# chenruduan/OAReactDiff

Hardware: AMD Instinct MI355X
Metric: denoising_steps_per_sec (higher is better)
Workload: dtype f32; 1 GPU; EGNNDynamics.forward (LEFTNet H=196 R=96 L=6), B=64 reactions/GPU x 3 objects x 23 atoms, complete graph per reaction (N=4416, E=300288), T=1000 sampler step shape; batch_per_gpu=64, atoms_per_object=23, parallelism=replica x1 (no collective), launch=eager

## Files before the change

oareactdiff_amd/_capi.py:

```python
from __future__ import annotations

import ctypes as C
import os

from .build import LIB

OARD_MAX_OBJECTS = 8
ABI_VERSION = 2041
OARD_OK, OARD_EINVAL, OARD_ENOTCOMPLETE, OARD_EHIP, OARD_ENOMEM = 0, -1, -2, -3, -4
ERRORS = {OARD_EINVAL: "invalid argument / unsupported configuration", OARD_ENOTCOMPLETE: "topology is not complete-per-sample",
          OARD_EHIP: "HIP runtime error", OARD_ENOMEM: "workspace too small"}

PREC_GCL_BF16X3, PREC_EQUI_BF16X3, PREC_TRAIN_BF16X3 = 1, 2, 4
TAP_S, TAP_VEC, TAP_EDGE, TAP_POS_FRAME, TAP_DPOS, TAP_HOUT, TAP_LABELS, TAP_NE1 = 1, 2, 3, 4, 5, 6, 7, 8

EXPORTS = ["oard_version", "oard_supported", "oard_param_count", "oard_packed_bytes", "oard_pack_weights",
           "oard_topology_create", "oard_topology_destroy", "oard_topology_num_nodes", "oard_topology_num_edges",
           "oard_topology_num_inner_edges", "oard_topology_num_samples", "oard_topology_check_edge_index",
           "oard_workspace_bytes", "oard_forward", "oard_active_inner_edges", "oard_debug_lin3u_table", "oard_sampler_step", "oard_sampler_step_dev", "oard_inpaint_step", "oard_inpaint_step_dev", "oard_tap", "oard_debug_stop_after", "oard_debug_option", "oard_timing_enable", "oard_timing_reset",
           "oard_timing_get",
           "oard_topology_create_parts", "oard_topology_export", "oard_tape_bytes", "oard_tape_entry", "oard_forward_train",
           "oard_packed_bwd_bytes", "oard_pack_weights_bwd", "oard_gcl_backward_dx", "oard_edge_node_sums",
           "oard_equi_backward_dx", "oard_scalarize_backward", "oard_equi_msg_backward", "oard_lin3u_forward", "oard_lin3u_backward", "oard_wgrad_scratch_bytes", "oard_wgrad",
           "oard_train_scratch_bytes", "oard_train_scratch_poison", "oard_train_scratch_entry", "oard_train_tail_backward",
           "oard_train_layer_backward", "oard_train_init_backward", "oard_train_stage_backward",
           "oard_loss_prepare", "oard_loss_terms", "oard_adamw_step", "oard_adamw_step_dev", "oard_nan_replace",
           "oard_adamw_step_ema", "oard_adamw_step_dev_ema", "oard_ema_update",
           "oard_graph_create", "oard_graph_destroy", "oard_graph_num_nodes", "oard_graph_num_edges", "oard_graph_object_rows",
           "oard_graph_is_complete", "oard_graph_workspace_bytes", "oard_graph_forward", "oard_library_stream"]
STAGE_RECOMPUTE, STAGE_UPDATE, STAGE_MESSAGE, STAGE_GCL_NODE, STAGE_NODE_PRE, STAGE_GCL_EDGE, STAGE_EQUI_EDGE = range(7)
SCRATCH_XH, SCRATCH_XQ, SCRATCH_CR, SCRATCH_DCD, SCRATCH_DCR = range(1, 6)

TOPO_NODE_REF, TOPO_NODE_OBJ, TOPO_NODE_ROW, TOPO_NODE_SAMPLE, TOPO_NODE_TIDX, TOPO_SAMPLE_PTR, TOPO_GROUP_PTR, \
    TOPO_INNER_SRC, TOPO_INNER_TGT, TOPO_ROW_SRC, TOPO_ROW_TGT = range(1, 12)
TAPE_HIN, TAPE_GEO, TAPE_RBF, TAPE_PP0, TAPE_X1 = 1, 2, 3, 4, 5
TAPE_S_IN, TAPE_VEC_IN, TAPE_EW, TAPE_AGG, TAPE_S_MID, TAPE_Z1, TAPE_Z2, TAPE_ATT, TAPE_Z3, TAPE_ZD1, TAPE_CD, TAPE_S_A, TAPE_VEC_A = range(16, 29)


class OardConfig(C.Structure):
    _fields_ = [
        ("hidden", C.c_int32), ("num_radial", C.c_int32), ("num_layers", C.c_int32), ("in_hidden", C.c_int32),
        ("n_obj", C.c_int32), ("node_nf", C.c_int32 * OARD_MAX_OBJECTS), ("enc_alias", C.c_int32 * OARD_MAX_OBJECTS),
        ("condition_nf", C.c_int32), ("condition_time", C.c_int32), ("pos_dim", C.c_int32), ("cutoff", C.c_float),
        ("reflect_equiv", C.c_int32), ("precision", C.c_int32),
    ]


class OardError(RuntimeError):
    pass


def check(rc: int, what: str) -> None:
    if rc != OARD_OK:
        raise OardError(f"{what} failed: {ERRORS.get(rc, rc)}")


def ptr_array(tensors, n=None):
    if tensors is None:
        return None
    ptrs = [None if t is None else t.data_ptr() for t in tensors]
    return (C.c_void_p * (len(ptrs) if n is None else n))(*ptrs)


_lib = None


def lib() -> C.CDLL:
    global _lib
    if _lib is not None:
        return _lib
    if not os.path.exists(LIB):
        raise OardError(f"{LIB} not found: build it with `python -m oareactdiff_amd.build` "
                        "(there is no CPU fallback for the HIP backend)")
    L = C.CDLL(LIB)
    vp, i32, i64, sz = C.c_void_p, C.c_int32, C.c_int64, C.c_size_t
    cfgp = C.POINTER(OardConfig)
    L.oard_version.restype = C.c_int
    got = L.oard_version()
    if got != ABI_VERSION:
        raise OardError(f"{LIB} has ABI version {got}, this package expects {ABI_VERSION}: rebuild it "
                        "(`python -m oareactdiff_amd.build --force`, or the script that made the OARD_LIB build)")
    L.oard_supported.argtypes = [cfgp]; L.oard_supported.restype = C.c_int
    L.oard_param_count.argtypes = [cfgp]; L.oard_param_count.restype = sz
    L.oard_packed_bytes.argtypes = [cfgp]; L.oard_packed_bytes.restype = sz
    L.oard_pack_weights.argtypes = [cfgp, C.POINTER(vp), sz, vp, sz, vp]; L.oard_pack_weights.restype = C.c_int
    L.oard_topology_create.argtypes = [cfgp, C.POINTER(i64), C.POINTER(i64), i64, C.POINTER(vp)]
    L.oard_topology_create.restype = C.c_int
    L.oard_topology_destroy.argtypes = [vp]; L.oard_topology_destroy.restype = None
    for f in ("oard_topology_num_nodes", "oard_topology_num_edges", "oard_topology_num_inner_edges",
              "oard_topology_num_samples"):
        getattr(L, f).argtypes = [vp]; getattr(L, f).restype = i64
    L.oard_topology_check_edge_index.argtypes = [vp, vp, i64, vp, vp]; L.oard_topology_check_edge_index.restype = C.c_int
    L.oard_workspace_bytes.argtypes = [cfgp, vp]; L.oard_workspace_bytes.restype = sz
    L.oard_forward.argtypes = [cfgp, vp, vp, C.POINTER(vp), vp, C.c_int, vp, C.POINTER(vp), vp, sz, vp, vp]
    L.oard_forward.restype = C.c_int
    L.oard_debug_lin3u_table.argtypes = [cfgp, vp, C.c_int, vp, vp]; L.oard_debug_lin3u_table.restype = C.c_int
    L.oard_active_inner_edges.argtypes = [cfgp, vp, vp, sz, C.POINTER(i64), vp]; L.oard_active_inner_edges.restype = C.c_int
    L.oard_sampler_step.argtypes = [cfgp, vp, C.c_int, C.POINTER(vp), C.POINTER(vp), C.POINTER(vp), C.POINTER(vp),
                                    C.c_float, C.c_float, C.c_float, C.c_int, C.POINTER(vp), vp]
    L.oard_sampler_step.restype = C.c_int
    L.oard_sampler_step_dev.argtypes = [cfgp, vp, C.c_int, C.POINTER(vp), C.POINTER(vp), C.POINTER(vp), C.POINTER(vp), vp, C.c_int,
                                        C.POINTER(vp), vp]
    L.oard_sampler_step_dev.restype = C.c_int
    pv = C.POINTER(vp)
    L.oard_inpaint_step.argtypes = [cfgp, vp, C.c_uint, pv, pv, pv, pv, pv, pv, pv, C.POINTER(C.c_float), C.c_int, pv, vp]
    L.oard_inpaint_step.restype = C.c_int
    L.oard_inpaint_step_dev.argtypes = [cfgp, vp, C.c_uint, pv, pv, pv, pv, pv, pv, pv, vp, C.c_int, pv, vp]
    L.oard_inpaint_step_dev.restype = C.c_int
    L.oard_tap.argtypes = [cfgp, vp, vp, C.c_int, C.c_int, vp, vp]; L.oard_tap.restype = C.c_int
    ci = C.c_int
    L.oard_topology_create_parts.argtypes = [cfgp, C.POINTER(i64), C.POINTER(i64), i64, ci, C.POINTER(vp)]
    L.oard_topology_create_parts.restype = ci
    L.oard_topology_export.argtypes = [vp, ci, vp, i64, vp]; L.oard_topology_export.restype = ci
    L.oard_tape_bytes.argtypes = [cfgp, vp]; L.oard_tape_bytes.restype = sz
    L.oard_tape_entry.argtypes = [cfgp, vp, ci, ci, C.POINTER(sz), C.POINTER(i64), C.POINTER(i64)]; L.oard_tape_entry.restype = ci
    L.oard_forward_train.argtypes = [cfgp, vp, vp, C.POINTER(vp), vp, ci, vp, C.POINTER(vp), vp, sz, vp, sz, vp, vp]
    L.oard_forward_train.restype = ci
    L.oard_packed_bwd_bytes.argtypes = [cfgp]; L.oard_packed_bwd_bytes.restype = sz
    L.oard_pack_weights_bwd.argtypes = [cfgp, C.POINTER(vp), sz, vp, sz, vp]; L.oard_pack_weights_bwd.restype = ci
    L.oard_gcl_backward_dx.argtypes = [cfgp, vp, vp, ci, vp, vp, vp, vp, vp, vp, vp, vp, vp]; L.oard_gcl_backward_dx.restype = ci
    L.oard_edge_node_sums.argtypes = [cfgp, vp, vp, vp, vp, vp]; L.oard_edge_node_sums.restype = ci
    L.oard_equi_backward_dx.argtypes = [cfgp, vp, vp, ci, vp, vp, vp, vp, vp]; L.oard_equi_backward_dx.restype = ci
    L.oard_scalarize_backward.argtypes = [cfgp, vp, vp, vp, vp, ci, vp, vp, vp, vp]; L.oard_scalarize_backward.restype = ci
    L.oard_equi_msg_backward.argtypes = [cfgp, vp, vp, ci, vp, vp, vp, vp, vp, vp, vp, vp, vp]; L.oard_equi_msg_backward.restype = ci
    L.oard_lin3u_forward.argtypes = [cfgp, vp, ci, vp, i64, vp, vp]; L.oard_lin3u_forward.restype = ci
    L.oard_lin3u_backward.argtypes = [cfgp, vp, ci, vp, vp, i64, vp, vp, vp, vp, vp, vp, vp]; L.oard_lin3u_backward.restype = ci
    L.oard_wgrad_scratch_bytes.argtypes = [ci, ci, i64]; L.oard_wgrad_scratch_bytes.restype = sz
    L.oard_wgrad.argtypes = [vp, ci, ci, ci, ci, ci, vp, ci, ci, ci, ci, ci, ci, i64, vp, vp, vp, sz, vp]; L.oard_wgrad.restype = ci
    pvp = C.POINTER(vp)
    L.oard_train_scratch_bytes.argtypes = [cfgp, vp]; L.oard_train_scratch_bytes.restype = sz
    L.oard_train_scratch_poison.argtypes = [cfgp, vp, vp, sz, vp]; L.oard_train_scratch_poison.restype = ci
    L.oard_train_scratch_entry.argtypes = [cfgp, vp, ci, C.POINTER(sz), C.POINTER(i64), C.POINTER(i64)]; L.oard_train_scratch_entry.restype = ci
    L.oard_train_tail_backward.argtypes = [cfgp, vp, vp, vp, vp, pvp, vp, vp, pvp, pvp, vp, sz, vp]; L.oard_train_tail_backward.restype = ci
    L.oard_train_layer_backward.argtypes = [cfgp, vp, vp, vp, vp, ci, vp, vp, vp, pvp, pvp, vp, sz, vp]; L.oard_train_layer_backward.restype = ci
    L.oard_train_init_backward.argtypes = [cfgp, vp, vp, vp, vp, pvp, vp, vp, pvp, pvp, vp, sz, vp]; L.oard_train_init_backward.restype = ci
    L.oard_train_stage_backward.argtypes = [cfgp, vp, vp, vp, vp, ci, ci, vp, vp, vp, vp, vp, vp, pvp, pvp, vp, sz, vp]
    L.oard_train_stage_backward.restype = ci
    L.oard_nan_replace.argtypes = [cfgp, vp, vp, pvp, pvp, vp]; L.oard_nan_replace.restype = ci
    pf, cf = C.POINTER(C.c_float), C.c_float
    L.oard_loss_prepare.argtypes = [cfgp, vp, pvp, pvp, pvp, pvp, vp, vp, ci, pf, pf, ci, ci, pvp, pvp, vp]; L.oard_loss_prepare.restype = ci
    L.oard_loss_terms.argtypes = [cfgp, vp, pvp, pvp, pvp, pvp, pvp, vp, vp, ci, pf, pf, pf, ci, ci, vp, vp, pvp, vp]; L.oard_loss_terms.restype = ci
    cd = C.c_double
    L.oard_adamw_step.argtypes = [vp, vp, vp, vp, vp, i64, cd, cd, cd, cd, cd, i64, ci, cd, vp]; L.oard_adamw_step.restype = ci
    L.oard_adamw_step_dev.argtypes = [vp, vp, vp, vp, vp, i64, cd, cd, cd, cd, cd, ci, ci, vp, ci, vp, vp, vp, vp]; L.oard_adamw_step_dev.restype = ci
    L.oard_adamw_step_ema.argtypes = [vp, vp, vp, vp, vp, i64, cd, cd, cd, cd, cd, i64, ci, cd, vp, cd, vp]; L.oard_adamw_step_ema.restype = ci
    L.oard_adamw_step_dev_ema.argtypes = [vp, vp, vp, vp, vp, i64, cd, cd, cd, cd, cd, ci, ci, vp, ci, vp, vp, vp, vp, cd, vp]
    L.oard_adamw_step_dev_ema.restype = ci
    L.oard_ema_update.argtypes = [vp, vp, i64, cd, vp]; L.oard_ema_update.restype = ci
    L.oard_library_stream.argtypes = [ci, pvp]; L.oard_library_stream.restype = ci
    L.oard_graph_create.argtypes = [cfgp, vp, vp, i64, vp, i64, pvp]; L.oard_graph_create.restype = ci
    L.oard_graph_destroy.argtypes = [vp]; L.oard_graph_destroy.restype = None
    L.oard_graph_num_nodes.argtypes = [vp]; L.oard_graph_num_nodes.restype = i64
    L.oard_graph_num_edges.argtypes = [vp]; L.oard_graph_num_edges.restype = i64
    L.oard_graph_object_rows.argtypes = [vp, ci]; L.oard_graph_object_rows.restype = i64
    L.oard_graph_is_complete.argtypes = [vp]; L.oard_graph_is_complete.restype = ci
    L.oard_graph_workspace_bytes.argtypes = [cfgp, vp]; L.oard_graph_workspace_bytes.restype = sz
    L.oard_graph_forward.argtypes = [cfgp, vp, pvp, sz, pvp, vp, ci, vp, pvp, vp, sz, vp, vp]; L.oard_graph_forward.restype = ci
    L.oard_debug_stop_after.argtypes = [C.c_int]; L.oard_debug_stop_after.restype = C.c_int
    L.oard_debug_option.argtypes = [C.c_char_p, C.c_int]; L.oard_debug_option.restype = C.c_int
    L.oard_timing_enable.argtypes = [C.c_int]; L.oard_timing_enable.restype = C.c_int
    L.oard_timing_reset.argtypes = []; L.oard_timing_reset.restype = C.c_int
    L.oard_timing_get.argtypes = [C.c_char_p, C.POINTER(C.c_double), C.POINTER(i64)]; L.oard_timing_get.restype = C.c_int
    for env, opt in (("OARD_GCL_VARIANT", b"gcl_variant"), ("OARD_EQUI_VARIANT", b"equi_variant"),
                     ("OARD_NODE_VARIANT", b"node_variant"), ("OARD_GCL_SKIP", b"gcl_skip"), ("OARD_EQUI_SKIP", b"equi_skip"), ("OARD_EQUI_L0_SKIP", b"equi_l0_skip"), ("OARD_EQUI_RBF_TABLE", b"equi_rbf_table"),("OARD_GCL_MSUM", b"gcl_msum"), ("OARD_GCL_PERSIST", b"gcl_persist"), ("OARD_GCL_GRID", b"gcl_grid"), ("OARD_PARTS", b"parts"), ("OARD_SEQUENTIAL", b"sequential"), ("OARD_POISON", b"poison"), ("OARD_AUTO_SMALL", b"auto_small"), ("OARD_AUTO_TINY", b"auto_tiny"), ("OARD_NPB", b"npb"),
                     ("OARD_WGRAD_WGS", b"wgrad_wgs"), ("OARD_WGRAD_LDS", b"wgrad_lds"), ("OARD_WGRAD_T16", b"wgrad_t16"), ("OARD_WGRAD_QUEUE", b"wgrad_queue"), ("OARD_GATE_FOLD", b"gate_fold"), ("OARD_WGRAD_SHAPES", b"wgrad_shapes"), ("OARD_TRAIN_DUAL", b"train_dual"), ("OARD_SMALL_SPLIT", b"small_split"),
                     ("OARD_SKIP_FAMILIES", b"skip_families")):
        if os.environ.get(env) not in (None, ""):
            check(L.oard_debug_option(opt, int(os.environ[env])), f"oard_debug_option({opt.decode()})")
    _lib = L
    return L


def timing_get(family: str):
    ms, n = C.c_double(0.0), C.c_int64(0)
    check(lib().oard_timing_get(family.encode(), C.byref(ms), C.byref(n)), "oard_timing_get")
    return ms.value, n.value
```

oareactdiff_amd/build.py:

```python
from __future__ import annotations

import os
import subprocess
import sys

CSRC = os.path.join(os.path.dirname(os.path.abspath(__file__)), "csrc")
LIB = os.environ.get("OARD_LIB") or os.path.join(CSRC, "liboard_hip.so")
_EDGE = ["oard_engine.h", "oard_layout.h", "oard_rbf_table.h", "oard_kernels.h", "oard_edge_v1.h", "oard_inst.h"]
SOURCES = {
    "oard_hip.hip": None,
    "oard_general.hip": ["oard_general.h"],
    "oard_inst_gcl_p.hip": _EDGE + ["oard_edge_p.h"],
    "oard_inst_gcl_v1.hip": _EDGE + ["oard_node_v1.h", "oard_edge_small.h"],
    "oard_inst_b3.hip": _EDGE + ["oard_edge_b3.h"],
    "oard_inst_equi.hip": _EDGE + ["oard_node_v1.h", "oard_edge_bwd.h"],
    "oard_inst_wgrad.hip": _EDGE + ["oard_edge_bwd.h", "oard_wgrad_t16.h"],
    "oard_inst_node.hip": _EDGE + ["oard_node_v1.h", "oard_edge_bwd.h", "oard_node_bwd.h", "oard_rows.h"],
}
_OWNED = {"oard_general.h"}
_PUBLIC = os.path.join("..", "..", "include", "oard.h")


def _deps(src):
    own = SOURCES[src]
    hdrs = sorted(f for f in os.listdir(CSRC) if f.endswith(".h") and f not in _OWNED) if own is None else list(own)
    return [src] + hdrs + [_PUBLIC]


def _objdir():
    return os.path.join(os.path.dirname(os.path.abspath(LIB)), "build", os.path.basename(LIB))


def _obj(src):
    return os.path.join(_objdir(), os.path.splitext(src)[0] + ".o")


def _newer(paths, than):
    if not os.path.exists(than):
        return True
    t = os.path.getmtime(than)
    return any(os.path.getmtime(os.path.join(CSRC, f)) > t for f in paths)


def _stale() -> bool:
    return any(_newer(_deps(src), LIB) for src in SOURCES)


DEFAULT_DIMS = "196x96,32x8,32x32"


def dims_define(spec: str) -> str:
    pairs = []
    for item in spec.replace(" ", "").split(","):
        if not item:
            continue
        h, r = item.lower().split("x")
        h, r = int(h), int(r)
        if h % 4 or r % 4 or h < 16 or r < 4:
            raise ValueError(f"OARD_DIMS entry {item!r}: widths must be multiples of 4 (hidden >= 16)")
        if (h, r) not in pairs:
            pairs.append((h, r))
    if not pairs:
        raise ValueError("OARD_DIMS is empty")
    return "-DOARD_DIMS_LIST=" + "".join(f"X({h},{r})" for h, r in pairs)


def _dims_file() -> str:
    return LIB + ".dims"


def _built_dims() -> str:
    try:
        with open(_dims_file()) as f:
            return f.read().strip()
    except OSError:
        return ""


def build(force: bool = False, verbose: bool = False) -> str:
    dims = os.environ.get("OARD_DIMS", DEFAULT_DIMS)
    dims_define(dims)
    if not force and not _stale() and _built_dims() == dims:
        return LIB
    hipcc = os.environ.get("HIPCC", "/opt/rocm/bin/hipcc")
    if not os.path.exists(hipcc):
        hipcc = "hipcc"
    os.makedirs(_objdir(), exist_ok=True)
    flags = ["--offload-arch=gfx950", "-O3", "-std=c++17", "-fPIC", "-Wno-unused-result", dims_define(dims)]
    extra = os.environ.get("OARD_CXXFLAGS", "").split()
    tag = os.path.join(_objdir(), "flags.txt")
    flag_line = " ".join(flags + extra)
    try:
        same_flags = open(tag).read() == flag_line
    except OSError:
        same_flags = False
    todo = [src for src in SOURCES if force or not same_flags or _newer(_deps(src), _obj(src))]

    def compile_one(src):
        cmd = [hipcc] + flags + extra + ["-c", src, "-o", _obj(src)]
        if verbose:
            print(" ".join(cmd), file=sys.stderr)
        subprocess.run(cmd, cwd=CSRC, check=True)
    if todo:
        from concurrent.futures import ThreadPoolExecutor
        with ThreadPoolExecutor(max_workers=len(todo)) as pool:
            list(pool.map(compile_one, todo))
        with open(tag, "w") as f:
            f.write(flag_line)
    cmd = [hipcc, "--offload-arch=gfx950", "-shared", "-fPIC"] + [_obj(src) for src in SOURCES] + ["-o", LIB]
    if verbose:
        print(" ".join(cmd), file=sys.stderr)
    subprocess.run(cmd, cwd=CSRC, check=True)
    with open(_dims_file(), "w") as f:
        f.write(dims + "\n")
    return LIB


if __name__ == "__main__":
    print(build(force="--force" in sys.argv, verbose=True))
```

oareactdiff_amd/csrc/oard_hip.hip:

```cpp
#include <algorithm>
#include <cmath>
#include <cstdio>
#include <cstring>
#include <map>
#include <string>
#include <vector>
#include <mutex>
#include <chrono>
#include <utility>

#include "oard_kernels.h"
#include "oard_edge_v1.h"
#include "oard_edge_p.h"
#include "oard_wgrad_t16.h"
#include "oard_edge_b3.h"
#ifdef OARD_EXPERIMENTS
#include "oard_edge_fp.h"
#endif
#include "oard_node_v1.h"
#include "oard_edge_small.h"
#include "oard_edge_bwd.h"
#include "oard_node_bwd.h"
#include "oard_rows.h"
#include "oard_plan.h"
#include "oard_inst.h"

#define OARD_VERSION 2041
#ifdef OARD_EXPERIMENTS
static constexpr bool kV0 = true;
#else
static constexpr bool kV0 = false;
#endif

#define HIP_TRY(x) do { hipError_t e_ = (x); if (e_ != hipSuccess) { \
    fprintf(stderr, "liboard_hip: %s failed: %s (%s:%d)\n", #x, hipGetErrorString(e_), __FILE__, __LINE__); \
    return OARD_EHIP; } } while (0)

namespace {
enum Family { F_GCL_EDGE = 0, F_EQUI_EDGE, F_NODE, F_INIT, F_OTHER, F_GCL_BWD, F_EQUI_BWD, F_WGRAD, F_COUNT };
const char* kFamilyNames[F_COUNT] = {"gcl_edge", "equi_edge", "node", "init", "other", "gcl_edge_bwd", "equi_edge_bwd", "wgrad"};
struct TimingRec { hipEvent_t a, b; int fam; };
struct Timing {
    bool on = false;
    std::vector<TimingRec> recs;
    std::vector<hipEvent_t> pool;
    double total_ms[F_COUNT] = {0};
    long long launches[F_COUNT] = {0};
    hipEvent_t get() {
        if (!pool.empty()) { hipEvent_t e = pool.back(); pool.pop_back(); return e; }
        hipEvent_t e; (void)hipEventCreate(&e); return e;
    }
    void flush() {
        for (auto& r : recs) {
            (void)hipEventSynchronize(r.b);
            float ms = 0.f;
            (void)hipEventElapsedTime(&ms, r.a, r.b);
            total_ms[r.fam] += ms; launches[r.fam] += 1;
            pool.push_back(r.a); pool.push_back(r.b);
        }
        recs.clear();
    }
} g_timing;
int g_stop_after = 0;
FwdOptions g_fwd;
int g_sequential = 0;
int g_npb = 0;
int g_poison = 0;
int g_gcl_msum_taken = 0;
int g_equi_l0_taken = 0;
int g_equi_rbf_taken = 0;
int g_parts = 0;
int g_wgrad_shapes = 3;
int g_wgrad_t16 = 256;
int g_wgrad_lds = 256;
int g_wgrad_wgs = 512;
int g_skip_families = 0;

struct ScopedLaunch {
    hipStream_t st; hipEvent_t a; int fam; bool on;
    ScopedLaunch(int f, hipStream_t s) : st(s), fam(f), on(g_timing.on) {
        if (on) { a = g_timing.get(); (void)hipEventRecord(a, st); }
    }
    ~ScopedLaunch() {
        if (on) { hipEvent_t b = g_timing.get(); (void)hipEventRecord(b, st); g_timing.recs.push_back({a, b, fam}); }
    }
};
#define LAUNCH(fam, kern, grid, block, stream, ...) do { ScopedLaunch sl_(fam, stream); if (!((g_skip_families >> (fam)) & 1)) \
    hipLaunchKernelGGL(kern, dim3((unsigned)(grid)), dim3(block), 0, stream, __VA_ARGS__); } while (0)
#define LAUNCH2(fam, kern, gx, gy, block, stream, ...) do { ScopedLaunch sl_(fam, stream); if (!((g_skip_families >> (fam)) & 1)) \
    hipLaunchKernelGGL(kern, dim3((unsigned)(gx), (unsigned)(gy)), dim3(block), 0, stream, __VA_ARGS__); } while (0)

#ifndef OARD_DIMS_LIST
#define OARD_DIMS_LIST X(196, 96) X(32, 8) X(32, 32)
#endif

inline size_t align_up(size_t x, size_t a) { return (x + a - 1) / a * a; }
inline long long cdiv(long long a, long long b) { return (a + b - 1) / b; }

bool config_ok(const oard_config* c) {
    if (!c) return false;
    bool dims = false;
#define X(h, r) dims = dims || (c->hidden == (h) && c->num_radial == (r));
    OARD_DIMS_LIST
#undef X
    if (!dims) return false;
    if (c->num_layers < 1 || c->num_layers > OARD_MAX_LAYERS) return false;
    if (c->in_hidden < 1 || c->in_hidden > 16) return false;
    if (c->n_obj < 1 || c->n_obj > OARD_MAX_OBJECTS) return false;
    if (c->pos_dim != 3 || (c->reflect_equiv != 0 && c->reflect_equiv != 1)) return false;
    if (c->precision & ~(OARD_PREC_GCL_BF16X3 | OARD_PREC_EQUI_BF16X3 | OARD_PREC_TRAIN_BF16X3)) return false;
    const int emb = c->in_hidden - (c->condition_time ? 1 : 0) - (c->condition_nf > 0 ? c->condition_nf : 0);
    if (emb < 1) return false;
    for (int k = 0; k < c->n_obj; ++k) {
        const int d = c->node_nf[k] - 3;
        if (d < 1 || d > 16) return false;
        const int a = c->enc_alias[k];
        if (a < 0 || a >= c->n_obj || c->node_nf[a] != c->node_nf[k]) return false;
    }
    return true;
}
int embed_dim(const oard_config* c) {
    return c->in_hidden - (c->condition_time ? 1 : 0) - (c->condition_nf > 0 ? c->condition_nf : 0);
}

PackOff make_layout(const oard_config* c) {
    const RDims d(c->hidden, c->num_radial);
    PackOff po;
    memset(&po, 0, sizeof(po));
    size_t cur = 0;
    auto take = [&](size_t n) { size_t o = cur; cur = align_up(cur + n, 64); return o; };
    auto mat = [&](int MT, int KB) { return take((size_t)MT * KB * 256); };
    const int emb = embed_dim(c);
    po.emb = mat(d.HT, 1); po.emb_b = take(d.HP);
    po.nbemb = mat(d.HT, 1); po.nbemb_b = take(d.HP);
    po.s2v = mat(d.HT, d.HT); po.s2v_b = take(d.HP);
    po.rl0 = mat(d.HT, d.RB); po.rl0_b = take(d.HP);
    po.rl2 = mat(d.HT, d.HT); po.rl2_b = take(d.HP);
    po.lin3 = take((size_t)d.H4 * 5 + 1);
    po.pe0 = take((size_t)d.H2 * 3);
    po.pe1 = mat(d.HT, d.PB);
    po.embout = mat(1, d.HT); po.embout_b = take(16);
    po.v1p = mat(d.HT, d.HT); po.v2p = take(d.HP);
    po.un0 = mat(d.HT, 2 * d.HT); po.un0_b = take(d.HP);
    po.un2 = mat(1, d.HT); po.un2_b = take(16);
    po.c0row = take(d.WP);
    po.u0 = take(d.HP);
    po.rbf_means = take(d.RP); po.rbf_betas = take(d.RP);
    for (int k = 0; k < c->n_obj; ++k) {
        const int dd = c->node_nf[k] - 3;
        po.enc[k] = take((size_t)2 * dd * dd + 2 * dd + (size_t)emb * 2 * dd + emb);
        po.dec[k] = take((size_t)2 * dd * emb + 2 * dd + (size_t)dd * 2 * dd + dd);
    }
    for (int l = 0; l < c->num_layers; ++l) {
        LayerOff& lo = po.layer[l];
        lo.ln_g_w = take(d.HP); lo.ln_g_b = take(d.HP);
        lo.W1a = mat(d.HT, d.HT); lo.b1 = take(d.HP);
        lo.W1b = mat(d.HT, d.HT);
        lo.W1c = mat(d.HT, d.WB);
        lo.W2 = mat(d.HT, d.HT); lo.b2 = take(d.HP);
        lo.watt = take(d.HP); lo.batt = take(1);
        lo.W3 = mat(d.WB, d.HT); lo.b3 = take(d.WP);
        lo.nm0 = mat(d.HT, 2 * d.HT); lo.nm0b = take(d.HP);
        lo.nm1 = mat(d.HT, d.HT); lo.nm1b = take(d.HP);
        lo.ln_q_w = take(d.HP); lo.ln_q_b = take(d.HP);
        lo.xp0 = mat(d.HT, d.HT);
        lo.xp2 = mat(3 * d.HT, d.HT);
        lo.dp0 = mat(d.D1T, d.WB); lo.dp0b = take(d.D1P);
        lo.dp2 = mat(3 * d.HT, d.D1T); lo.dp2b = take(3 * d.HP);
        lo.rbfp = mat(3 * d.HT, d.RB);
        lo.rbfw = take((size_t)3 * d.H * d.R); lo.rbff = take(4);
        lo.vp = mat(2 * d.HT, d.HT);
        lo.xv0 = mat(d.HT, 2 * d.HT);
        lo.xv2 = mat(3 * d.HT, d.HT);
        lo.l3u = take(593);
        lo.l3t = take(L3T_FLOATS);
        lo.gcl_stream = take((size_t)(d.WB * d.HT + (d.HT + 1) * (d.HT + 1) + d.WB * (d.HT + 1)) * 256);
        lo.equi_stream = take((size_t)(d.WB * d.D1T + 3 * d.HT * (1 + d.D1T + d.RB)) * 256);
        {
            const int nbh = (d.HT + 1) / 2, nbw = (d.WB + 1) / 2;
            lo.gcl_b3 = take((size_t)(nbw * 3 * d.HT + (d.HT + 1) * (1 + 3 * nbh) + d.WB * (1 + 3 * nbh)) * 256);
            lo.equi_b3 = take((size_t)(nbw * 3 * d.D1T + ((d.RB + 1) / 2 + (d.D1T + 1) / 2) * 9 * d.HT) * 256);
        }
    }
    po.head = cur;
    for (int l = 0; l < c->num_layers; ++l) po.layer[l].rbft = take(rbt_layer_floats(d.HT));
    po.total = cur;
    po.signed_scal = c->reflect_equiv ? 0 : 1;
    for (int l = 0; l < c->num_layers; ++l) po.layer[l].xcross = c->reflect_equiv ? 0 : 1;
    return po;
}

struct ParamIdx {
    int emb_w, emb_b, embout_w, embout_b, means, betas, nbemb_w, nbemb_b, s2v_w, s2v_b, rl0_w, rl0_b, rl2_w, rl2_b,
        lin30_w, lin30_b, lin32_w, lin32_b, pe0_w, pe1_w;
    int gcl0, msg0, upd0, out0, enc0, dec0, count;
    explicit ParamIdx(const oard_config* c) {
        int i = 0;
        emb_w = i++; emb_b = i++; embout_w = i++; embout_b = i++; means = i++; betas = i++;
        nbemb_w = i++; nbemb_b = i++; s2v_w = i++; s2v_b = i++; rl0_w = i++; rl0_b = i++; rl2_w = i++; rl2_b = i++;
        lin30_w = i++; lin30_b = i++; lin32_w = i++; lin32_b = i++; pe0_w = i++; pe1_w = i++;
        i += 2;
        gcl0 = i; i += 14 * c->num_layers;
        msg0 = i; i += 9 * c->num_layers;
        upd0 = i; i += 9 * c->num_layers;
        i += 2;
        out0 = i; i += 6;
        enc0 = i; i += 4 * c->n_obj;
        dec0 = i; i += 4 * c->n_obj;
        count = i;
    }
};

struct Packer {
    const float* const* p; float* blob; hipStream_t st;
    std::vector<GenJob> jobs;
    long long blocks = 0;
    void push(GenJob j, size_t work) {
        j.block0 = blocks;
        blocks += cdiv((long long)std::max<size_t>(work, 1), 256);
        jobs.push_back(j);
    }
    void matrix(int src, int src_ld, int col_off, int msl, int msp, int ms, int ksl, int ksp, int ks, int MT, int KB,
                size_t dst, size_t tstride = 0, size_t bstride = 256, int perm_ht = 0, int transpose = 0, int tail_compact = 0,
                int rows4 = 0) {
        if (tstride == 0) tstride = (size_t)KB * 256;
        GenJob j;
        memset(&j, 0, sizeof(j));
        j.type = 0;
        j.m = PackJob{p[src], src_ld, col_off, msl, msp, ms, ksl, ksp, ks, MT, KB, dst, tstride, bstride, perm_ht, transpose, rows4, tail_compact};
        push(j, (size_t)MT * KB * 256);
    }
    void nat(int src, int src_ld, int col_off, int M, int K, int MT, int KB, size_t dst) {
        matrix(src, src_ld, col_off, M, MT * 16, 1, K, KB * 16, 1, MT, KB, dst);
    }
    void vec(int src, int sect_len, int sect_pad, int sects, int n_dst, size_t dst) {
        GenJob j;
        memset(&j, 0, sizeof(j));
        j.type = 1; j.src = src >= 0 ? p[src] : nullptr; j.dst = dst; j.sect_len = sect_len; j.sect_pad = sect_pad; j.sects = sects; j.n = n_dst;
        push(j, (size_t)n_dst);
    }
    void bias_chunks(int src, int sect_len, int sect_pad, int sects, int n_tiles, size_t dst, size_t tstride,
                     int perm_ht = 0) {
        GenJob j;
        memset(&j, 0, sizeof(j));
        j.type = 2; j.src = p[src]; j.dst = dst; j.sect_len = sect_len; j.sect_pad = sect_pad; j.sects = sects; j.n = n_tiles * 256;
        j.tstride = tstride; j.perm_ht = perm_ht;
        push(j, (size_t)n_tiles * 256);
    }
    void raw(int src, int n, size_t dst) {
        GenJob j;
        memset(&j, 0, sizeof(j));
        j.type = 3; j.src = p[src]; j.dst = dst; j.n = n;
        push(j, (size_t)n);
    }
    int flush() {
        if (jobs.empty()) return OARD_OK;
        struct Cached { std::vector<GenJob> host; GenJob* dev = nullptr; size_t cap = 0; };
        static std::mutex mu;
        static std::map<std::pair<const void*, int>, Cached> cache;
        int devid = 0;
        (void)hipGetDevice(&devid);
        const GenJob* table = nullptr;
        {
            std::lock_guard<std::mutex> lk(mu);
            Cached& c = cache[{(const void*)blob, devid}];
            const bool same = c.host.size() == jobs.size() && memcmp(c.host.data(), jobs.data(), jobs.size() * sizeof(GenJob)) == 0;
            if (!same) {
                HIP_TRY(hipStreamSynchronize(st));
                if (c.cap < jobs.size()) {
                    if (c.dev) (void)hipFree(c.dev);
                    HIP_TRY(hipMalloc((void**)&c.dev, jobs.size() * sizeof(GenJob)));
                    c.cap = jobs.size();
                }
                HIP_TRY(hipMemcpy(c.dev, jobs.data(), jobs.size() * sizeof(GenJob), hipMemcpyHostToDevice));
                c.host = jobs;
            }
            table = c.dev;
        }
        hipLaunchKernelGGL(k_pack_all, dim3((unsigned)blocks), dim3(256), 0, st, table, (int)jobs.size(), blob);
        jobs.clear();
        blocks = 0;
        return OARD_OK;
    }
};
struct RbfTablesOf { const void* blob; unsigned good; };
static std::mutex g_rbf_mu;
static std::vector<RbfTablesOf> g_rbf_known;
static void rbf_tables_forget(const void* blob) {
    std::lock_guard<std::mutex> lk(g_rbf_mu);
    g_rbf_known.erase(std::remove_if(g_rbf_known.begin(), g_rbf_known.end(), [&](const RbfTablesOf& e) { return e.blob == blob; }), g_rbf_known.end());
}
static int rbf_tables_for(const oard_config* c, const PackOff& po, const float* blob, hipStream_t st, unsigned* good) {
    *good = 0;
    std::lock_guard<std::mutex> lk(g_rbf_mu);
    for (const RbfTablesOf& e : g_rbf_known) if (e.blob == blob) { *good = e.good; return OARD_OK; }
    hipStreamCaptureStatus cap = hipStreamCaptureStatusNone;
    HIP_TRY(hipStreamIsCapturing(st, &cap));
    if (cap != hipStreamCaptureStatusNone) return OARD_OK;
    const RDims d(c->hidden, c->num_radial);
    RbtJobs j;
    memset(&j, 0, sizeof(j));
    for (int l = 0; l < c->num_layers; ++l) { j.w[l] = po.layer[l].rbfw; j.tab[l] = po.layer[l].rbft; j.flag[l] = po.layer[l].rbff; }
    j.means = po.rbf_means; j.betas = po.rbf_betas; j.H = d.H; j.HT = d.HT; j.R = d.R;
    hipLaunchKernelGGL(k_rbf_table_fill, dim3((unsigned)cdiv((long long)3 * d.HT * (RBT_N + 1) * 4, 256), (unsigned)c->num_layers), dim3(256), 0, st,
                       const_cast<float*>(blob), j);
    hipLaunchKernelGGL(k_rbf_table_check, dim3((unsigned)(3 * d.HT * 4), (unsigned)c->num_layers), dim3(256), 0, st, const_cast<float*>(blob), j);
    HIP_TRY(hipGetLastError());
    std::vector<float> flags((size_t)c->num_layers, 0.f);
    for (int l = 0; l < c->num_layers; ++l)
        HIP_TRY(hipMemcpyAsync(&flags[l], blob + po.layer[l].rbff, sizeof(float), hipMemcpyDeviceToHost, st));
    HIP_TRY(hipStreamSynchronize(st));
    unsigned mask = 0;
    for (int l = 0; l < c->num_layers; ++l) if (flags[l] == 1.0f) mask |= 1u << l;
    if (g_rbf_known.size() >= 64) g_rbf_known.erase(g_rbf_known.begin());
    g_rbf_known.push_back({blob, mask});
    *good = mask;
    return OARD_OK;
}

#define OARD_SMALL_MAX_EDGES (512 * 16 * 16)
static WsOff make_ws(const oard_config* c, const TopoDev& td) {
    const RDims d(c->hidden, c->num_radial);
    const size_t N = td.N, E = td.E + 1, A = td.A + 1;
    WsOff w;
    size_t cur = 0;
    auto take = [&](size_t bytes) { size_t o = cur; cur = align_up(cur + bytes, 256); return o; };
    w.pos = take(N * 3 * 4); w.pf64 = take(N * 3 * 8); w.pf32 = take(N * 3 * 4); w.x1 = take(N * 3 * 4);
    w.pp0 = take(N * 4); w.labels = take(N * 4); w.hin = take(N * 16 * 4);
    w.zemb = take(N * d.HP * 4); w.nb = take(N * d.HP * 4); w.s = take(N * d.HP * 4); w.s1 = take(N * d.HP * 4);
    w.ne1 = take(N * 3 * d.HP * 4); w.xh = take(N * d.HP * 4); w.P = take(N * d.HP * 4); w.Q = take(N * d.HP * 4);
    w.xq = take(N * 3 * d.HP * 4); w.vec = take(N * 3 * d.HP * 4); w.vec2 = take(N * 3 * d.HP * 4); w.v2buf = take(N * 3 * d.HP * 4);
    w.sc0 = take(N * d.HP * 4); w.vdot = take(N * d.HP * 4);
    w.geo = take(A * GEO_STRIDE * 4); w.d64 = take(A * 8); w.rbuf = take(A * d.RP * 4);
    w.ew = take(E * d.WP * 4); w.mbuf = take(std::max(E, (size_t)(td.CI + td.CX) + 1) * d.HP * 4);
    w.xmsg = take(A * d.HP * 4); w.vmsg = take(A * 3 * d.HP * 4);
    w.dpos = take(N * 3 * 4); w.hout = take(N * 16 * 4);
    w.al_rows = take(A * 4); w.al_src = take(A * 4); w.al_pre = take(A * 4); w.al_cnt = take((size_t)cdiv((long long)td.A, 256) * 4 + 4); w.al_n = take(4);
    w.d1s = take((size_t)cdiv((long long)td.A, 128) * 8 * d.D1T * 1024);
    w.small_a = E <= (size_t)OARD_SMALL_MAX_EDGES ? take(A * d.D1P * 4) : 0;
    w.rbt = take(A * RBT_ROW * 4);
    w.total = cur;
    return w;
}



template <class K>
int set_lds(K kernel, size_t bytes) {
    HIP_TRY(hipFuncSetAttribute((const void*)kernel, hipFuncAttributeMaxDynamicSharedMemorySize, (int)bytes));
    return OARD_OK;
}

#define LAUNCH_LDS(fam, kern, grid, block, lds, stream, ...) do { \
    static bool attr_done_[64] = {}; \
    int dev_ = 0; (void)hipGetDevice(&dev_); dev_ &= 63; \
    if (!attr_done_[dev_]) { int rc_ = set_lds(kern, lds); if (rc_ != OARD_OK) return rc_; attr_done_[dev_] = true; } \
    ScopedLaunch sl_(fam, stream); if (!((g_skip_families >> (fam)) & 1)) \
    hipLaunchKernelGGL(kern, dim3((unsigned)(grid)), dim3(block), lds, stream, __VA_ARGS__); } while (0)

static int device_cus() {
    static int cus[64] = {};
    int d = 0;
    (void)hipGetDevice(&d);
    d &= 63;
    if (!cus[d]) {
        int n = 0;
        if (hipDeviceGetAttribute(&n, hipDeviceAttributeMultiprocessorCount, d) != hipSuccess || n < 1) { (void)hipGetLastError(); n = 256; }
        cus[d] = n;
    }
    return cus[d];
}
struct GclArgs {
    const TopoDev& tp; const float* wb; const LayerOff& lo;
    const float *stream, *P, *Q, *u0, *c0; float *ew_in, *ew_out, *mbuf;
    GclTape tape; hipStream_t st;
};
template <class D, bool S1, bool S3>
int launch_gcl_v1s(const GclLaunch& L, bool msum, const GclArgs& a) {
    constexpr size_t RING3 = GclStream<D, 2>::LDS_BYTES / 2 * 3;
#define GCL_STREAMED(kern, waves, lds, w_) do { LAUNCH_LDS(F_GCL_EDGE, kern, L.grid, (waves) * 64, lds, a.st, a.tp, w_, a.P, a.Q, a.u0, a.c0, \
                                                           L.r0, L.r1, a.ew_in, a.ew_out, a.mbuf, a.tape); return OARD_OK; } while (0)
    switch ((int)L.shape) {
        case GCL_PERSIST:
            if (msum) GCL_STREAMED((k_gcl_edge_p<D, S1, S3, false, true>), 8, RING3, a.stream);
            GCL_STREAMED((k_gcl_edge_p<D, S1, S3>), 8, RING3, a.stream);
        case GCL_RING3:
            if (msum) GCL_STREAMED((k_gcl_edge_v1<D, 8, 2, S1, S3, false, true, 2, 3>), 8, RING3, a.stream);
            GCL_STREAMED((k_gcl_edge_v1<D, 8, 2, S1, S3, false, false, 2, 3>), 8, RING3, a.stream);
        case GCL_TRAIN_PERSIST: GCL_STREAMED((k_gcl_edge_p<D, S1, S3, true>), 8, RING3, a.stream);
        case GCL_TRAIN_RING3: GCL_STREAMED((k_gcl_edge_v1<D, 8, 2, S1, S3, true, false, 2, 3>), 8, RING3, a.stream);
        case GCL_B3: GCL_STREAMED((k_gcl_edge_b3<D, S1, S3>), 8, (GclB3Stream<D>::LDS_BYTES), a.wb + a.lo.gcl_b3);
        case GCL_TRAIN_B3: GCL_STREAMED((k_gcl_edge_b3<D, S1, S3, true>), 8, (GclB3Stream<D>::LDS_BYTES), a.wb + a.lo.gcl_b3);
        case GCL_W4: GCL_STREAMED((k_gcl_edge_v1<D, 4, 2, S1, S3, false>), 4, (GclStream<D, 2>::LDS_BYTES), a.stream);
        case GCL_SMALL:
            LAUNCH_LDS(F_GCL_EDGE, (k_gcl_edge_small<D, 8, S1, S3>), L.grid, 512, (GclSmall<D>::LDS_BYTES), a.st,
                       a.tp, a.wb, a.lo, a.P, a.Q, a.u0, a.c0, L.r0, L.r1, a.ew_out, a.mbuf);
            return OARD_OK;
#ifdef OARD_EXPERIMENTS
        case GCL_V0: LAUNCH(F_GCL_EDGE, (k_gcl_edge<D>), L.grid, 256, a.st, a.tp, a.wb, a.lo, a.P, a.Q, a.ew_in, a.mbuf); return OARD_OK;
        case GCL_X0 + 7: GCL_STREAMED((k_gcl_edge_v1<D, 8, 2, S1, S3, false>), 8, (GclStream<D, 2>::LDS_BYTES), a.stream);
        case GCL_X0 + 8: GCL_STREAMED((k_gcl_edge_v1<D, 8, 3, S1, S3, false>), 8, (GclStream<D, 3>::LDS_BYTES), a.stream);
        case GCL_X0 + 9: GCL_STREAMED((k_gcl_edge_v1<D, 8, 4, S1, S3, false>), 8, (GclStream<D, 4>::LDS_BYTES), a.stream);
        case GCL_X0 + 4: GCL_STREAMED((k_gcl_edge_fp<D, 8, 2, S1, S3, false>), 8, (GclRing<D, 2, 4>::LDS_BYTES), a.stream);
        case GCL_X0 + 5: GCL_STREAMED((k_gcl_edge_fp<D, 8, 2, S1, S3, false, 3>), 8, (GclRing<D, 2, 3>::LDS_BYTES), a.stream);
        case GCL_X0 + 10: GCL_STREAMED((k_gcl_edge_v1<D, 12, 1, S1, S3, false, false, 3>), 12, (GclStream<D, 1>::LDS_BYTES), a.stream);
        case GCL_X0 + 11: GCL_STREAMED((k_gcl_edge_v1<D, 12, 2, S1, S3, false, false, 3>), 12, (GclStream<D, 2>::LDS_BYTES), a.stream);
        case GCL_X0 + 12: GCL_STREAMED((k_gcl_edge_v1<D, 4, 1, S1, S3, false, false, 3>), 4, (GclStream<D, 1>::LDS_BYTES), a.stream);
#endif
        default: return OARD_EINVAL;
    }
#undef GCL_STREAMED
}
template <class D>
int launch_gcl_v1(const GclLayer& g, bool msum, const GclArgs& a) {
    for (int i = 0; i < g.n; ++i) {
        const GclLaunch& L = g.l[i];
        const int rc = L.s1 ? (L.s3 ? launch_gcl_v1s<D, true, true>(L, msum, a) : launch_gcl_v1s<D, true, false>(L, msum, a))
                            : (L.s3 ? launch_gcl_v1s<D, false, true>(L, msum, a) : launch_gcl_v1s<D, false, false>(L, msum, a));
        if (rc != OARD_OK) return rc;
    }
    return OARD_OK;
}
template <class D>
int launch_equi_v1(const FwdPlan& plan, int l, const TopoDev& tp, const float* wb, const LayerOff& lo, const float* stream, const float* dp0b,
                   const float* ew, const float* rbuf, float* qbuf, float* zd1, float* cd, hipStream_t st, float* d1s, float* small, ActList al,
                   const float* rbt) {
    const long long tiles = cdiv(tp.A, 16);
    switch (plan.equi) {
        case EQ_TRAIN_B3:
            LAUNCH_LDS(F_EQUI_EDGE, (k_equi_edge_b3<D, true>), cdiv(tp.A, 16 * 8), 8 * 64, (EquiB3Stream<D>::LDS_BYTES), st, tp, wb + lo.equi_b3,
                       dp0b, wb + lo.dp2b, ew, rbuf, qbuf, d1s, zd1, cd, ActList{});
            return OARD_OK;
        case EQ_TRAIN:
            LAUNCH_LDS(F_EQUI_EDGE, (k_equi_edge_v1<D, 8, true>), cdiv(tp.A, 16 * 8), 8 * 64, (EquiStream<D>::LDS_BYTES), st,
                       tp, stream, dp0b, ew, rbuf, qbuf, zd1, cd, ActList{}, 0, (const float*)nullptr);
            return OARD_OK;
        case EQ_SMALL_SPLIT:
            LAUNCH_LDS(F_EQUI_EDGE, (k_equi_small_s1<D, 8>), tiles * cdiv(D::D1T, 8), 512, (size_t)D::WB * 1024, st, tp, wb, lo, ew, small);
            LAUNCH_LDS(F_EQUI_EDGE, (k_equi_small_s2<D, 8>), tiles * cdiv(3 * D::HT, 8), 512, (size_t)(D::D1T + D::RB) * 1024, st,
                       tp, wb, lo, (const float*)small, rbuf, qbuf);
            return OARD_OK;
        case EQ_SMALL:
            LAUNCH_LDS(F_EQUI_EDGE, (k_equi_edge_small<D, 8>), tiles, 512, (EquiSmall<D>::LDS_BYTES), st, tp, wb, lo, ew, rbuf, qbuf);
            return OARD_OK;
        case EQ_B3:
            LAUNCH_LDS(F_EQUI_EDGE, (k_equi_edge_b3<D>), cdiv(tp.A, 16 * 8), 8 * 64, (EquiB3Stream<D>::LDS_BYTES), st, tp, wb + lo.equi_b3,
                       dp0b, wb + lo.dp2b, ew, rbuf, qbuf, d1s, nullptr, nullptr, al);
            return OARD_OK;
        case EQ_W4:
            LAUNCH_LDS(F_EQUI_EDGE, (k_equi_edge_v1<D, 4, false>), cdiv(tp.A, 16 * 4), 4 * 64, (EquiStream<D>::LDS_BYTES), st,
                       tp, stream, dp0b, ew, rbuf, qbuf, nullptr, nullptr, al, 0, (const float*)nullptr);
            return OARD_OK;
        case EQ_W8:
            if (plan.rbf_table[l])
                LAUNCH_LDS(F_EQUI_EDGE, (k_equi_edge_v1<D, 8, false, true>), cdiv(tp.A, 16 * 8), 8 * 64, (EquiStream<D>::LDS_BYTES), st,
                           tp, stream, dp0b, ew, rbt, qbuf, nullptr, nullptr, al, plan.l0_skip && l == 0 ? 1 : 0, wb + lo.rbft);
            else
                LAUNCH_LDS(F_EQUI_EDGE, (k_equi_edge_v1<D, 8, false>), cdiv(tp.A, 16 * 8), 8 * 64, (EquiStream<D>::LDS_BYTES), st,
                           tp, stream, dp0b, ew, rbuf, qbuf, nullptr, nullptr, al, plan.l0_skip && l == 0 ? 1 : 0, (const float*)nullptr);
            return OARD_OK;
        default: return OARD_EINVAL;
    }
}

struct TapeOff {
    size_t hin, geo, rbuf, pp0, x1;
    size_t s_in[OARD_MAX_LAYERS + 1], vec_in[OARD_MAX_LAYERS + 1];
    size_t agg[OARD_MAX_LAYERS], s_mid[OARD_MAX_LAYERS];
    size_t s_a[OARD_MAX_LAYERS], vec_a[OARD_MAX_LAYERS];
    size_t ew[OARD_MAX_LAYERS + 1];
    size_t z1[OARD_MAX_LAYERS], z2[OARD_MAX_LAYERS], att[OARD_MAX_LAYERS], z3[OARD_MAX_LAYERS];
    size_t zd1[OARD_MAX_LAYERS], cd[OARD_MAX_LAYERS];
    size_t total;
};
static TapeOff make_tape(const oard_config* c, const TopoDev& td) {
    const RDims d(c->hidden, c->num_radial);
    const size_t N = td.N, E = td.E + 1, A = td.A + 1;
    TapeOff t;
    memset(&t, 0, sizeof(t));
    size_t cur = 0;
    auto take = [&](size_t bytes) { size_t o = cur; cur = align_up(cur + bytes, 256); return o; };
    t.hin = take(N * 16 * 4); t.geo = take(A * GEO_STRIDE * 4); t.rbuf = take(A * d.RP * 4); t.pp0 = take(N * 4); t.x1 = take(N * 3 * 4);
    for (int l = 0; l <= c->num_layers; ++l) {
        t.s_in[l] = take(N * d.HP * 4); t.vec_in[l] = take(N * 3 * d.HP * 4); t.ew[l] = take(E * d.WP * 4);
        if (l == c->num_layers) break;
        t.agg[l] = take(N * d.HP * 4); t.s_mid[l] = take(N * d.HP * 4);
        t.s_a[l] = take(N * d.HP * 4); t.vec_a[l] = take(N * 3 * d.HP * 4);
        t.z1[l] = take(E * d.HP * 4); t.z2[l] = take(E * d.HP * 4); t.att[l] = take(E * 4); t.z3[l] = take(E * d.WP * 4);
        t.zd1[l] = take(A * d.D1P * 4); t.cd[l] = take(A * 3 * d.HP * 4);
    }
    t.total = cur;
    return t;
}

template <class D>
static int forward_impl(const FwdOptions& opt, const oard_config* c, const TopoPart* topo, const float* wb, const float* const* xh,
                        const float* t, int t_scalar, const float* cond, float* const* out, char* ws, char* tape,
                        int* status, hipStream_t st) {
    const TopoDev& tp = topo->d;
    const PackOff po = make_layout(c);
    const WsOff w = make_ws(c, tp);
    const bool train = tape != nullptr;
    const TapeOff to = train ? make_tape(c, tp) : TapeOff{};
    const int emb = embed_dim(c);
    float* pos = (float*)(ws + w.pos); double* pf64 = (double*)(ws + w.pf64); float* pf32 = (float*)(ws + w.pf32);
    auto slot = [&](size_t ws_off, size_t tape_off) -> float* { return train ? (float*)(tape + tape_off) : (float*)(ws + ws_off); };
    float* x1 = slot(w.x1, to.x1); float* pp0 = slot(w.pp0, to.pp0); int* labels = (int*)(ws + w.labels);
    float* hin = slot(w.hin, to.hin); float* zemb = (float*)(ws + w.zemb); float* nb = (float*)(ws + w.nb);
    float* s = (float*)(ws + w.s); float* s1 = (float*)(ws + w.s1); float* ne1 = (float*)(ws + w.ne1);
    float* xhb = (float*)(ws + w.xh); float* P = (float*)(ws + w.P); float* Q = (float*)(ws + w.Q);
    float* xq = (float*)(ws + w.xq); float* vec = slot(w.vec, to.vec_in[0]); float* v2buf = (float*)(ws + w.v2buf);
    float* scal = (float*)(ws + w.sc0); float* vdot = (float*)(ws + w.vdot);
    float* geo = slot(w.geo, to.geo); double* d64 = (double*)(ws + w.d64); float* rbuf = slot(w.rbuf, to.rbuf);
    float* mbuf = (float*)(ws + w.mbuf); float* xmsg = (float*)(ws + w.xmsg);
    float* vmsg = (float*)(ws + w.vmsg); float* dpos = (float*)(ws + w.dpos); float* hout = (float*)(ws + w.hout);
    auto ew_at = [&](int l) -> float* { return train ? (float*)(tape + to.ew[l]) : (float*)(ws + w.ew); };
    float* ew = ew_at(0);
    auto s_at = [&](int l) -> float* { return train ? (float*)(tape + to.s_in[l]) : s; };
    auto s_mid_at = [&](int l) -> float* { return train ? (float*)(tape + to.s_mid[l]) : s; };

    ObjPtrs op;
    memset(&op, 0, sizeof(op));
    for (int k = 0; k < c->n_obj; ++k) {
        op.xh[k] = xh[k]; op.out[k] = out[k]; op.node_nf[k] = c->node_nf[k]; op.enc[k] = po.enc[k]; op.dec[k] = po.dec[k];
    }
    const long long N = tp.N, E = tp.E, A = tp.A;
    const unsigned gN = (unsigned)cdiv(N, 64), gA = (unsigned)cdiv(A, 64);
    const double cutoff = (double)c->cutoff;
    FwdPlanIn plan_in{opt, c->precision, train, topo->conc, tp.npb, device_cus(), A, E, tp.CI, tp.CX, c->num_layers, w.small_a != 0};
    if (plan_rbf_wanted(plan_in)) { const int rc = rbf_tables_for(c, po, wb, st, &plan_in.rbf_good); if (rc != OARD_OK) return rc; }
    const FwdPlan plan = make_fwd_plan(plan_in);
    bool any_rbt = false, all_rbt = c->num_layers > 0;
    for (int l = 0; l < c->num_layers; ++l) { any_rbt = any_rbt || plan.rbf_table[l]; all_rbt = all_rbt && plan.rbf_table[l]; }
    g_equi_rbf_taken = all_rbt;
    const bool msum = plan.msum, use_al = plan.use_al, nv1 = plan.node != NODE_V0;
    const int stop_after = train ? 0 : g_stop_after;
    int* al_cnt = (int*)(ws + w.al_cnt);
    const ActList al = use_al ? ActList{(const int*)(ws + w.al_rows), (const int*)(ws + w.al_src), (const int*)(ws + w.al_pre), (const int*)(ws + w.al_n)}
                              : ActList{nullptr, nullptr, nullptr, nullptr};
    if (!use_al) HIP_TRY(hipMemsetAsync(ws + w.al_n, 0xff, sizeof(int), st));
    LAUNCH(F_OTHER, k_prep, cdiv(N, 128), 128, st, tp, op, wb, pos, hin, t, t_scalar, cond,
           c->condition_nf > 0 ? c->condition_nf : 0, c->condition_time, emb);
    LAUNCH(F_INIT, k_geom, tp.n_groups, 64, st, tp, (const float*)pos, cutoff, pf64, pf32, x1, pp0, labels);
    if (plan.fill_edges || stop_after == 1)
        LAUNCH(F_INIT, k_fill_edges, std::min<long long>(cdiv((E - A + 1) * (D::WP / 4), 256), 8192), 256, st,
               wb + po.c0row, ew + (size_t)A * D::WP, E - A + 1, D::WP);
    if (A > 0) {
        LAUNCH(F_INIT, k_edge_geo, cdiv(A, 256), 256, st, tp, (const float*)pos, (const double*)pf64, cutoff, geo, d64, use_al ? al_cnt : nullptr);
        if (use_al) LAUNCH(F_INIT, k_active_list, cdiv(A, 256), 256, st, tp, (const float*)geo, (const int*)al_cnt, (int*)al.rows, (int*)al.src, (int*)al.pre, (int*)al.n);
        LAUNCH(F_INIT, k_rbf, cdiv(A * D::RP, 256), 256, st, tp, (const double*)d64, (const float*)geo,
               wb + po.rbf_means, wb + po.rbf_betas, cutoff, rbuf, ew, D::R, D::RP, D::H, D::WP, any_rbt ? (float*)(ws + w.rbt) : (float*)nullptr);
    }
    LAUNCH(F_INIT, (k_node_embed<D>), gN, 256, st, tp, wb, po, (const float*)hin, zemb, nb);
    if (A > 0) LAUNCH(F_INIT, (k_radial_lin<D>), gA, 256, st, tp, wb, po, (const float*)rbuf, (const float*)geo, ew);
    constexpr int NW = D::HT <= 16 ? D::HT : 8;
    const unsigned gNb = (unsigned)cdiv(N, tp.npb);
    if (plan.init_v1) {
        LAUNCH(F_INIT, (k_neighbor_v1<D, NW>), gNb, NW * 64, st, tp, wb, po, (const float*)zemb, (const float*)nb, (const float*)ew, s_at(0), s1);
        LAUNCH(F_INIT, (k_s2v_agg_v1<D, NW>), gNb, NW * 64, st, tp, (const float*)s1, (const float*)ew, (const float*)geo, ne1);
    } else if constexpr (kV0) {
        LAUNCH(F_INIT, (k_neighbor<D>), gN, 256, st, tp, wb, po, (const float*)zemb, (const float*)nb, (const float*)ew, s_at(0), s1);
        LAUNCH(F_INIT, (k_s2v_agg<D>), gN, 256, st, tp, (const float*)s1, (const float*)ew, (const float*)geo, ne1);
    } else return OARD_EINVAL;
    if (A > 0) LAUNCH2(F_INIT, (k_scalarize<D>), gA, (plan.scalarize_tiles ? D::HT : 1), 256, st, tp, wb, po, (const float*)ne1, (const float*)geo, ew);
    HIP_TRY(hipMemsetAsync(vec, 0, (size_t)N * 3 * D::HP * sizeof(float), st));
    if (stop_after == 1) return OARD_OK;

    float* vec2 = (float*)(ws + w.vec2);
    float* vcur = vec;
    float* vnext = vec2;
    g_gcl_msum_taken = msum;
    for (int l = 0; l < c->num_layers; ++l) {
        const LayerOff lo = po.layer[l];
        const unsigned gN16 = (unsigned)cdiv(N, tp.npb);
        float* ew_in = ew_at(l);
        float* ew_out = ew_at(l + 1);
        if (train) vnext = (float*)(tape + to.vec_in[l + 1]);

        if (nv1) LAUNCH(F_NODE, (k_node_pre_v1<D, NW>), gN16, NW * 64, st, tp, wb, po, lo, (const float*)s_at(l), (const float*)pp0, xhb, P, Q);
        else if constexpr (kV0) LAUNCH(F_NODE, (k_node_pre<D>), gN, 256, st, tp, wb, po, lo, (const float*)s, (const float*)pp0, xhb, P, Q);
        else return OARD_EINVAL;
        GclTape gt{};
        if (train) gt = GclTape{(float*)(tape + to.z1[l]), (float*)(tape + to.z2[l]), (float*)(tape + to.att[l]), (float*)(tape + to.z3[l])};
        int rc = launch_gcl_v1<D>(plan.gcl_at(l), msum, GclArgs{tp, wb, lo, wb + lo.gcl_stream, P, Q, wb + po.u0, wb + po.c0row, ew_in, ew_out, mbuf, gt, st});
        if (rc != OARD_OK) return rc;
        const bool rows = plan.node == NODE_ROWS;
        if (nv1 && rows) LAUNCH(F_NODE, (k_gcl_node_v1<D, NW, true>), gN16, NW * 64, st, tp, wb, lo, (const float*)xhb, (const float*)mbuf, s_mid_at(l), xq,
                                train ? (float*)(tape + to.agg[l]) : nullptr);
        else if (nv1 && msum) LAUNCH(F_NODE, (k_gcl_node_v1<D, NW, false, true>), gN16, NW * 64, st, tp, wb, lo, (const float*)xhb, (const float*)mbuf, s_mid_at(l), xq,
                                     (float*)nullptr);
        else if (nv1) LAUNCH(F_NODE, (k_gcl_node_v1<D, NW, false>), gN16, NW * 64, st, tp, wb, lo, (const float*)xhb, (const float*)mbuf, s_mid_at(l), xq,
                             train ? (float*)(tape + to.agg[l]) : nullptr);
        else if constexpr (kV0) LAUNCH(F_NODE, (k_gcl_node<D>), gN, 256, st, tp, wb, lo, (const float*)xhb, (const float*)mbuf, s, xq);
        else return OARD_EINVAL;
        if (stop_after == 100 + 10 * l + 1) { topo->vec_final = (size_t)((char*)vcur - ws); return OARD_OK; }
        if (plan.equi == EQ_V0) {
            if constexpr (kV0) {
                if (A > 0) LAUNCH(F_EQUI_EDGE, (k_equi_edge<D>), gA, 256, st, tp, wb, lo, (const float*)ew_out, (const float*)rbuf,
                                  (const float*)geo, (const float*)xq, (const float*)vcur, xmsg, vmsg);
                LAUNCH(F_NODE, (k_equi_agg<D>), gN, 256, st, tp, wb, lo, (const float*)xmsg, (const float*)vmsg, (const float*)x1,
                       s, vcur, v2buf, scal, vdot);
            } else return OARD_EINVAL;
        } else {
            const bool l0_skip = l == 0 && plan.l0_skip;
            if (l == 0) g_equi_l0_taken = l0_skip;
            if (A > 0) {
                rc = launch_equi_v1<D>(plan, l, tp, wb, lo, wb + lo.equi_stream, wb + lo.dp0b, ew_out, rbuf, vmsg,
                                       train ? (float*)(tape + to.zd1[l]) : nullptr, train ? (float*)(tape + to.cd[l]) : nullptr, st,
                                       (float*)(ws + w.d1s), (float*)(ws + w.small_a), al, (const float*)(ws + w.rbt));
                if (rc != OARD_OK) return rc;
            }
#define EQUI_NODE_V1(D_, ROWS_, XC_) LAUNCH(F_NODE, (k_equi_node_v1<D_, NW, ROWS_, XC_>), gN16, NW * 64, st, tp, wb, lo, (const float*)vmsg, \
                       (const float*)xq, (const float*)geo, (const float*)x1, (const float*)s_mid_at(l), s_at(l + 1), (const float*)vcur, vnext, \
                       train ? (float*)(tape + to.s_a[l]) : nullptr, train ? (float*)(tape + to.vec_a[l]) : nullptr, al)
            if (nv1 && rows) {
                if (lo.xcross) EQUI_NODE_V1(D, true, true); else EQUI_NODE_V1(D, true, false);
            } else if (nv1 && l0_skip) {
                if (lo.xcross) EQUI_NODE_V1(Layer0<D>, false, true); else EQUI_NODE_V1(Layer0<D>, false, false);
            } else if (nv1) {
                if (lo.xcross) EQUI_NODE_V1(D, false, true); else EQUI_NODE_V1(D, false, false);
            } else if constexpr (kV0) {
                LAUNCH(F_NODE, (k_equi_agg_v1<D>), gN, 256, st, tp, wb, lo, (const float*)vmsg, (const float*)xq,
                       (const float*)geo, (const float*)x1, s, (const float*)vcur, vnext, v2buf, scal, vdot);
            } else return OARD_EINVAL;
            std::swap(vcur, vnext);
        }
        if constexpr (kV0) {
            if (!nv1) LAUNCH(F_NODE, (k_equi_upd<D>), gN, 256, st, tp, wb, lo, (const float*)scal, (const float*)vdot,
                             (const float*)v2buf, s, vcur);
        }
        if (stop_after == 100 + 10 * l + 2) { topo->vec_final = (size_t)((char*)vcur - ws); return OARD_OK; }
    }
    if (!train) topo->vec_final = (size_t)((char*)vcur - ws);
    if (train) {
        ZeroRows z;
        z.count = 0;
        auto add = [&](size_t off, size_t row, int ld) {
            if (z.count == 64) { LAUNCH(F_OTHER, k_zero_rows, 64, 256, st, z); z.count = 0; }
            z.p[z.count] = (float*)(tape + off) + row * (size_t)ld; z.n[z.count] = ld; ++z.count;
        };
        for (int l = 0; l <= c->num_layers; ++l) {
            add(to.ew[l], (size_t)E, D::WP);
            if (l == c->num_layers) break;
            add(to.z1[l], (size_t)E, D::HP); add(to.z2[l], (size_t)E, D::HP); add(to.att[l], (size_t)E, 1); add(to.z3[l], (size_t)E, D::WP);
            add(to.zd1[l], (size_t)A, D::D1P); add(to.cd[l], (size_t)A, 3 * D::HP);
        }
        add(to.geo, (size_t)A, GEO_STRIDE); add(to.rbuf, (size_t)A, D::RP);
        if (z.count > 0) LAUNCH(F_OTHER, k_zero_rows, z.count, 256, st, z);
    }
    if (plan.init_v1)
        LAUNCH(F_NODE, (k_out_v1<D, NW>), gNb, NW * 64, st, tp, wb, po, (const float*)s_at(c->num_layers), (const float*)vcur, dpos, hout, status);
    else if constexpr (kV0)
        LAUNCH(F_NODE, (k_out<D>), gN, 256, st, tp, wb, po, (const float*)s, (const float*)vcur, dpos, hout, status);
    else return OARD_EINVAL;
    LAUNCH(F_OTHER, k_post, cdiv(N, 128), 128, st, tp, op, wb, (const float*)dpos, (const float*)hout, emb);
    HIP_TRY(hipGetLastError());
    return OARD_OK;
}

template <class F> static int dispatch_dims(const oard_config* c, F&& f) {
#define X(h, r) if (c->hidden == (h) && c->num_radial == (r)) { f(Dims<(h), (r)>{}); return 0; }
    OARD_DIMS_LIST
#undef X
    return OARD_EINVAL;
}
#define DISPATCH_DIMS(c, CALL)                                                                         \
    do {                                                                                               \
        if (dispatch_dims((c), [&](auto d_) { using D = decltype(d_); CALL; }) != 0) return OARD_EINVAL; \
    } while (0)

struct BwdLayerOff { size_t gcl, equi, watt; };
struct BwdOff { BwdLayerOff layer[OARD_MAX_LAYERS]; size_t total; };
static BwdOff make_bwd_layout(const oard_config* c) {
    const RDims d(c->hidden, c->num_radial);
    BwdOff b;
    memset(&b, 0, sizeof(b));
    size_t cur = 0;
    auto take = [&](size_t n) { size_t o = cur; cur = align_up(cur + n, 64); return o; };
    for (int l = 0; l < c->num_layers; ++l) {
        b.layer[l].gcl = take((size_t)(2 * d.WB * d.HT + d.HT * d.HT) * 256);
        b.layer[l].equi = take((size_t)(3 * d.HT * d.D1T + d.WB * d.D1T) * 256);
        b.layer[l].watt = take(d.HP);
    }
    b.total = cur;
    return b;
}
template <class D>
static int gcl_backward_impl(const oard_config* c, const TopoDev& tp, const float* pb, const BwdLayerOff& bl, int layer,
                             const char* tape, const TapeOff& to, const float* dagg, float* dew, float* dz3, float* mout,
                             float* dz2, float* da, float* dz1, hipStream_t st, float* gate_part = nullptr, long long* gate_rows = nullptr) {
    GclBwdArgs a;
    a.gate_part = gate_part;
    a.z1 = (const float*)(tape + to.z1[layer]); a.z2 = (const float*)(tape + to.z2[layer]);
    a.att = (const float*)(tape + to.att[layer]); a.z3 = (const float*)(tape + to.z3[layer]);
    a.dagg = dagg; a.watt = pb + bl.watt; a.dew = dew; a.dz3 = dz3; a.mout = mout; a.dz2 = dz2; a.da = da; a.dz1 = dz1;
    const float* stream = pb + bl.gcl;
    const bool last = layer == c->num_layers - 1;
    const long long r_full = last ? tp.A : tp.E;
    long long rows = 0;
    if (r_full > 0) {
        LAUNCH_LDS(F_GCL_BWD, (k_gcl_edge_bwd<D, 8, 2, true>), cdiv(r_full, 128), 512, (GclBwdStream<D, 2>::LDS_BYTES), st,
                   tp, stream, 0LL, r_full, a);
        rows += cdiv(r_full, 128) * 8;
    }
    if (last && tp.E > tp.A) {
        if (a.gate_part) a.gate_part += (size_t)rows * D::HP;
        LAUNCH_LDS(F_GCL_BWD, (k_gcl_edge_bwd<D, 8, 2, false>), cdiv(tp.E - tp.A, 128), 512, (GclBwdStream<D, 2>::LDS_BYTES), st,
                   tp, stream, tp.A, tp.E, a);
        rows += cdiv(tp.E - tp.A, 128) * 8;
    }
    if (gate_rows) *gate_rows = rows;
    HIP_TRY(hipGetLastError());
    return OARD_OK;
}

template <class D>
static int equi_backward_impl(const TopoDev& tp, const float* stream, const float* dcd, const float* zd1, float* dew,
                              float* dzd1, hipStream_t st) {
    LAUNCH_LDS(F_EQUI_BWD, (k_equi_edge_bwd<D, 8>), cdiv(tp.A, 128), 512, (EquiBwdStream<D>::LDS_BYTES), st, tp, stream, dcd,
               zd1, dew, dzd1);
    HIP_TRY(hipGetLastError());
    return OARD_OK;
}

#ifndef OARD_SCAL_BWD_WAVES
#define OARD_SCAL_BWD_WAVES 2
#endif
template <class D>
static int scalarize_backward_impl(const oard_config* c, const TopoDev& tp, const float* wb, const char* tape, const TapeOff& to,
                                   const float* ne1, int ld, const float* dew, float* dne1, float* part, hipStream_t st) {
    const PackOff po = make_layout(c);
    constexpr int NW = OARD_SCAL_BWD_WAVES;
    if (po.signed_scal)
        LAUNCH(F_INIT, (k_scalarize_bwd<D, NW, true>), tp.N, NW * 64, st, tp, wb + po.lin3, ne1, ld, (const float*)(tape + to.geo), dew, dne1, part);
    else
        LAUNCH(F_INIT, (k_scalarize_bwd<D, NW, false>), tp.N, NW * 64, st, tp, wb + po.lin3, ne1, ld, (const float*)(tape + to.geo), dew, dne1, part);
    HIP_TRY(hipGetLastError());
    return OARD_OK;
}

template <class D>
static int equi_msg_backward_impl(const oard_config* c, const TopoDev& tp, const char* tape, const TapeOff& to, int layer, const float* xq, const float* cr,
                                  const float* gs, const float* gv, float* dcd, float* dcr, float* dxq, float* dvec, hipStream_t st) {
    const Strided3 xq3{xq, 3 * D::H, D::H}, vec3{(const float*)(tape + to.vec_in[layer]), 3 * D::HP, D::HP}, cr3{cr, 3 * D::H, D::H},
        gv3{gv, 3 * D::H, D::H};
    LAUNCH(F_NODE, (k_equi_msg_bwd<D>), tp.N, 256, st, tp, (const float*)(tape + to.geo), xq3, vec3, (const float*)(tape + to.cd[layer]), cr3,
           gs, D::H, gv3, dcd, dcr, dxq, dvec, D::H, c->reflect_equiv ? 0 : 1);
    HIP_TRY(hipGetLastError());
    return OARD_OK;
}

struct WgradPlan { int transposed, NT, nPB, nQG, PP, QP, gy; long long rpc; int n_chunks; int lds, PBW, QGW; };
struct WglShape { int NT, PBW, QGW; };
static const WglShape kWglShapes[2] = {{7, 4, 2}, {8, 4, 2}};
static WgradPlan wgrad_plan(int ncY, int ncX, long long rows) {
    WgradPlan p;
    p.transposed = ncX > ncY ? 1 : 0;
    const int ncP = p.transposed ? ncX : ncY, ncQ = p.transposed ? ncY : ncX;
    const int nQT = (int)cdiv(ncQ, 16);
    p.NT = (cdiv(nQT, 7) * 7 <= cdiv(nQT, 8) * 8) ? 7 : 8;
    p.nPB = (int)cdiv(ncP, 64); p.nQG = (int)cdiv(nQT, p.NT);
    p.PP = p.nPB * 64; p.QP = p.nQG * p.NT * 16;
    p.gy = (int)cdiv((long long)p.nPB * p.nQG, 4);
    long long want = std::max<long long>(1, g_wgrad_wgs / p.gy);
    want = std::min(want, std::max<long long>(1, cdiv(rows, rows < 16384 ? 128 : 64)));
    p.rpc = align_up((size_t)cdiv(std::max<long long>(rows, 1), want), 4 * OARD_WG_PD);
    p.n_chunks = (int)cdiv(std::max<long long>(rows, 1), p.rpc);
    p.lds = 0; p.PBW = 4; p.QGW = 2;
    if (g_wgrad_lds > 0 && rows >= 16384) {
        long long best = -1;
        for (int k = 0; k < 2; ++k) {
            if (!((g_wgrad_shapes >> k) & 1)) continue;
            const WglShape& c = kWglShapes[k];
            const long long nQG = cdiv(nQT, c.NT);
            if (nQG < 2) continue;
            const long long sP = cdiv(p.nPB, c.PBW) * c.PBW, sQ = cdiv(nQG, c.QGW) * c.QGW;
            if ((long long)p.nPB * nQG * 20 < sP * sQ * 17) continue;
            const long long cost = sP * 64 * sQ * c.NT * 16;
            if (best < 0 || cost < best) { best = cost; p.lds = 1; p.NT = c.NT; p.PBW = c.PBW; p.QGW = c.QGW; p.nQG = (int)nQG; }
        }
        if (p.lds) p.QP = p.nQG * p.NT * 16;
    }
    if (p.lds) {
        const long long tiles = cdiv(p.nPB, p.PBW) * cdiv(p.nQG, p.QGW);
        long long w2 = std::max<long long>(1, g_wgrad_lds / tiles);
        w2 = std::min(w2, std::max<long long>(1, cdiv(rows, 4 * WGL_ROWS)));
        p.rpc = align_up((size_t)cdiv(rows, w2), WGL_ROWS);
        p.n_chunks = (int)cdiv(rows, p.rpc);
        p.gy = (int)tiles;
    }
    return p;
}
}

extern "C" {

int oard_version(void) { return OARD_VERSION; }
int oard_supported(const oard_config* cfg) { return config_ok(cfg) ? OARD_OK : OARD_EINVAL; }
size_t oard_param_count(const oard_config* cfg) { return config_ok(cfg) ? (size_t)ParamIdx(cfg).count : 0; }
size_t oard_packed_bytes(const oard_config* cfg) { return config_ok(cfg) ? make_layout(cfg).total * sizeof(float) : 0; }

int oard_pack_weights(const oard_config* c, const float* const* params, size_t n_params, void* packed,
                      size_t packed_bytes, oard_stream_t stream) {
    if (!config_ok(c) || !params || !packed) return OARD_EINVAL;
    const ParamIdx pi(c);
    if (n_params != (size_t)pi.count) return OARD_EINVAL;
    const PackOff po = make_layout(c);
    if (packed_bytes < po.total * sizeof(float)) return OARD_ENOMEM;
    const RDims d(c->hidden, c->num_radial);
    const int H = d.H, R = d.R, W = d.W, C = c->in_hidden, emb = embed_dim(c);
    hipStream_t st = (hipStream_t)stream;
    rbf_tables_forget(packed);
    HIP_TRY(hipMemsetAsync(packed, 0, po.head * sizeof(float), st));
    Packer pk{params, (float*)packed, st, {}, 0};

    pk.nat(pi.emb_w, C, 0, H, C, d.HT, 1, po.emb);          pk.vec(pi.emb_b, H, d.HP, 1, d.HP, po.emb_b);
    pk.nat(pi.nbemb_w, C, 0, H, C, d.HT, 1, po.nbemb);      pk.vec(pi.nbemb_b, H, d.HP, 1, d.HP, po.nbemb_b);
    pk.nat(pi.s2v_w, H, 0, H, H, d.HT, d.HT, po.s2v);       pk.vec(pi.s2v_b, H, d.HP, 1, d.HP, po.s2v_b);
    pk.nat(pi.rl0_w, R, 0, H, R, d.HT, d.RB, po.rl0);       pk.vec(pi.rl0_b, H, d.HP, 1, d.HP, po.rl0_b);
    pk.nat(pi.rl2_w, H, 0, H, H, d.HT, d.HT, po.rl2);       pk.vec(pi.rl2_b, H, d.HP, 1, d.HP, po.rl2_b);
    pk.raw(pi.lin30_w, d.H4 * 3, po.lin3);
    pk.raw(pi.lin30_b, d.H4, po.lin3 + d.H4 * 3);
    pk.raw(pi.lin32_w, d.H4, po.lin3 + d.H4 * 4);
    pk.raw(pi.lin32_b, 1, po.lin3 + d.H4 * 5);
    pk.raw(pi.pe0_w, d.H2 * 3, po.pe0);
    pk.nat(pi.pe1_w, d.H2, 0, H, d.H2, d.HT, d.PB, po.pe1);
    pk.nat(pi.embout_w, H, 0, C, H, 1, d.HT, po.embout);    pk.vec(pi.embout_b, C, 16, 1, 16, po.embout_b);
    pk.raw(pi.means, R, po.rbf_means);                      pk.raw(pi.betas, R, po.rbf_betas);
    const int o = pi.out0;
    pk.nat(o + 0, H, 0, H, H, d.HT, d.HT, po.v1p);
    pk.vec(o + 1, H, d.HP, 1, d.HP, po.v2p);
    pk.matrix(o + 2, 2 * H, 0, H, d.HP, 1, H, d.HP, 2, d.HT, 2 * d.HT, po.un0);   pk.vec(o + 3, H, d.HP, 1, d.HP, po.un0_b);
    pk.nat(o + 4, H, 0, 2, H, 1, d.HT, po.un2);                                  pk.vec(o + 5, 2, 16, 1, 16, po.un2_b);
    for (int k = 0; k < c->n_obj; ++k) {
        const int a = c->enc_alias[k], dd = c->node_nf[k] - 3;
        const int e = pi.enc0 + 4 * a, q = pi.dec0 + 4 * a;
        size_t off = po.enc[k];
        pk.raw(e + 0, 2 * dd * dd, off); off += 2 * dd * dd;
        pk.raw(e + 1, 2 * dd, off); off += 2 * dd;
        pk.raw(e + 2, emb * 2 * dd, off); off += emb * 2 * dd;
        pk.raw(e + 3, emb, off);
        off = po.dec[k];
        pk.raw(q + 0, 2 * dd * emb, off); off += 2 * dd * emb;
        pk.raw(q + 1, 2 * dd, off); off += 2 * dd;
        pk.raw(q + 2, dd * 2 * dd, off); off += dd * 2 * dd;
        pk.raw(q + 3, dd, off);
    }
    for (int l = 0; l < c->num_layers; ++l) {
        const LayerOff& lo = po.layer[l];
        const int g = pi.gcl0 + 14 * l;
        const int ld0 = 2 * H + W;
        pk.nat(g + 0, ld0, 0, H, H, d.HT, d.HT, lo.W1a);     pk.vec(g + 1, H, d.HP, 1, d.HP, lo.b1);
        pk.nat(g + 0, ld0, H, H, H, d.HT, d.HT, lo.W1b);
        pk.nat(g + 0, ld0, 2 * H, H, W, d.HT, d.WB, lo.W1c);
        pk.nat(g + 2, H, 0, H, H, d.HT, d.HT, lo.W2);        pk.vec(g + 3, H, d.HP, 1, d.HP, lo.b2);
        pk.matrix(g + 4, 2 * H, 0, H, d.HP, 1, H, d.HP, 2, d.HT, 2 * d.HT, lo.nm0);   pk.vec(g + 5, H, d.HP, 1, d.HP, lo.nm0b);
        pk.nat(g + 6, H, 0, H, H, d.HT, d.HT, lo.nm1);       pk.vec(g + 7, H, d.HP, 1, d.HP, lo.nm1b);
        pk.nat(g + 8, H, 0, W, H, d.WB, d.HT, lo.W3);        pk.vec(g + 9, W, d.WP, 1, d.WP, lo.b3);
        pk.vec(g + 10, H, d.HP, 1, d.HP, lo.watt);           pk.raw(g + 11, 1, lo.batt);
        pk.vec(g + 12, H, d.HP, 1, d.HP, lo.ln_g_w);         pk.vec(g + 13, H, d.HP, 1, d.HP, lo.ln_g_b);
        const int m = pi.msg0 + 9 * l;
        pk.nat(m + 0, W, 0, 3 * H, W, d.D1T, d.WB, lo.dp0);   pk.vec(m + 1, 3 * H, d.D1P, 1, d.D1P, lo.dp0b);
        pk.matrix(m + 2, 3 * H, 0, H, d.HP, 3, 3 * H, d.D1P, 1, 3 * d.HT, d.D1T, lo.dp2);
        pk.vec(m + 3, H, d.HP, 3, 3 * d.HP, lo.dp2b);
        pk.nat(m + 4, H, 0, H, H, d.HT, d.HT, lo.xp0);
        pk.matrix(m + 5, H, 0, H, d.HP, 3, H, d.HP, 1, 3 * d.HT, d.HT, lo.xp2);
        pk.matrix(m + 6, R, 0, H, d.HP, 3, R, d.RP, 1, 3 * d.HT, d.RB, lo.rbfp);
        pk.raw(m + 6, 3 * H * R, lo.rbfw);
        pk.vec(m + 7, H, d.HP, 1, d.HP, lo.ln_q_w);          pk.vec(m + 8, H, d.HP, 1, d.HP, lo.ln_q_b);
        const int u = pi.upd0 + 9 * l;
        pk.matrix(u + 0, H, 0, H, d.HP, 2, H, d.HP, 1, 2 * d.HT, d.HT, lo.vp);
        pk.matrix(u + 1, 2 * H, 0, H, d.HP, 1, H, d.HP, 2, d.HT, 2 * d.HT, lo.xv0);
        pk.matrix(u + 2, H, 0, H, d.HP, 3, H, d.HP, 1, 3 * d.HT, d.HT, lo.xv2);
        pk.raw(u + 3, 144, lo.l3u); pk.raw(u + 4, 48, lo.l3u + 144); pk.raw(u + 5, 384, lo.l3u + 192);
        pk.raw(u + 6, 8, lo.l3u + 576); pk.raw(u + 7, 8, lo.l3u + 584); pk.raw(u + 8, 1, lo.l3u + 592);
        {
            const size_t G2 = (size_t)(d.HT + 1) * 256;
            const size_t s1 = lo.gcl_stream, s2 = s1 + (size_t)d.WB * d.HT * 256, s3 = s2 + (size_t)(d.HT + 1) * G2;
            const int tc = (H % 16 >= 1 && H % 16 <= 4 && d.HT >= 3 && (d.HT & 1)) ? 1 : 0;
            pk.matrix(g + 0, ld0, 2 * H, H, d.HP, 1, W, d.WP, 1, d.HT, d.WB, s1, 256, (size_t)d.HT * 256, 0, 0, 0, tc * d.HT);
            pk.matrix(g + 2, H, 0, H, d.HP, 1, H, d.HP, 1, d.HT, d.HT, s2 + 256, G2, 256, 0, 0, tc, tc * d.HT);
            pk.bias_chunks(g + 3, H, d.HP, 1, d.HT, s2, G2);
            pk.matrix(g + 10, H, 0, 1, 16, 1, H, d.HP, 1, 1, d.HT, s2 + d.HT * G2 + 256, G2, 256, 0, 0, tc, tc);
            pk.bias_chunks(g + 11, 1, 16, 1, 1, s2 + d.HT * G2, G2);
            pk.matrix(g + 8, H, 0, W, d.WP, 1, H, d.HP, 1, d.WB, d.HT, s3 + 256, G2, 256, 0, 0, tc);
            pk.bias_chunks(g + 9, W, d.WP, 1, d.WB, s3, G2);
            const size_t GE = (size_t)(1 + d.D1T + d.RB) * 256;
            const size_t t1 = lo.equi_stream, t2 = t1 + (size_t)d.WB * d.D1T * 256;
            pk.matrix(m + 0, W, 0, 3 * H, d.D1P, 1, W, d.WP, 1, d.D1T, d.WB, t1, 256, (size_t)d.D1T * 256);
            const int r4 = (H % 16 >= 1 && H % 16 <= 4) ? d.HT : 0;
            pk.matrix(m + 2, 3 * H, 0, H, d.HP, 3, 3 * H, d.D1P, 1, 3 * d.HT, d.D1T, t2 + 256, GE, 256, d.HT, 0, 0, r4);
            pk.matrix(m + 6, R, 0, H, d.HP, 3, R, d.RP, 1, 3 * d.HT, d.RB, t2 + (size_t)(1 + d.D1T) * 256, GE, 256, d.HT, 0, 0, r4);
            pk.bias_chunks(m + 3, H, d.HP, 3, 3 * d.HT, t2, GE, d.HT);
        }
    }
    { int rcf = pk.flush(); if (rcf != OARD_OK) return rcf; }
    {
        L3tJobs lj;
        memset(&lj, 0, sizeof(lj));
        for (int l = 0; l < c->num_layers; ++l) { lj.l3u[l] = po.layer[l].l3u; lj.l3t[l] = po.layer[l].l3t; }
        hipLaunchKernelGGL(k_lin3u_table_fill, dim3(L3T_N / 256, (unsigned)c->num_layers), dim3(256), 0, st, (float*)packed, lj);
        hipLaunchKernelGGL(k_lin3u_table_check, dim3(L3T_N / 256, (unsigned)c->num_layers), dim3(256), 0, st, (float*)packed, lj);
    }
    hipLaunchKernelGGL(k_c0row, dim3((unsigned)cdiv(d.WP, 256)), dim3(256), 0, st, params[pi.lin30_b], params[pi.lin32_w],
                       params[pi.lin32_b], params[pi.rl0_b], params[pi.rl2_w], params[pi.rl2_b],
                       (float*)packed + po.c0row, H, d.H4, d.WP);
    hipLaunchKernelGGL(k_u0, dim3((unsigned)cdiv(d.HP, 64)), dim3(64), 0, st, params[pi.gcl0 + 0],
                       (const float*)packed + po.c0row, (float*)packed + po.u0, H, W, d.HP);
    if (c->precision & (OARD_PREC_GCL_BF16X3 | OARD_PREC_TRAIN_BF16X3)) {
        const int nbh = (d.HT + 1) / 2, nbw = (d.WB + 1) / 2, G1 = 3 * d.HT, G2 = 1 + 3 * nbh;
        const size_t G2f = (size_t)(d.HT + 1) * 256;
        for (int l = 0; l < c->num_layers; ++l) {
            const LayerOff& lo = po.layer[l];
            const size_t s1 = lo.gcl_b3, s2 = s1 + (size_t)nbw * G1 * 256, s3 = s2 + (size_t)(d.HT + 1) * G2 * 256;
            const size_t f2 = lo.gcl_stream + (size_t)d.WB * d.HT * 256, f3 = f2 + (size_t)(d.HT + 1) * G2f;
            B3Jobs jb;
            jb.j[0] = B3Job{lo.W1c, d.WB, d.HT, nbw, 0, s1, (size_t)3 * 256, (size_t)G1 * 256};
            jb.j[1] = B3Job{lo.W2, d.HT, d.HT, nbh, 0, s2 + 256, (size_t)G2 * 256, (size_t)3 * 256};
            jb.j[2] = B3Job{lo.watt, d.HT, 1, nbh, 1, s2 + (size_t)d.HT * G2 * 256 + 256, (size_t)G2 * 256, (size_t)3 * 256};
            jb.j[3] = B3Job{lo.W3, d.HT, d.WB, nbh, 0, s3 + 256, (size_t)G2 * 256, (size_t)3 * 256};
            const long long work = std::max<long long>((long long)d.HT * nbw, (long long)d.WB * nbh) * 64;
            hipLaunchKernelGGL(k_pack_b3, dim3((unsigned)cdiv(work, 256), 4), dim3(256), 0, st, jb, (float*)packed);
            hipLaunchKernelGGL(k_copy_chunks, dim3((unsigned)(d.HT + 1)), dim3(256), 0, st, (float*)packed, f2, G2f, s2, (size_t)G2 * 256, d.HT + 1);
            hipLaunchKernelGGL(k_copy_chunks, dim3((unsigned)d.WB), dim3(256), 0, st, (float*)packed, f3, G2f, s3, (size_t)G2 * 256, d.WB);
        }
    }
    if (c->precision & (OARD_PREC_EQUI_BF16X3 | OARD_PREC_TRAIN_BF16X3)) {
        const int nbw = (d.WB + 1) / 2, nbr = (d.RB + 1) / 2, nbd = (d.D1T + 1) / 2, NO = 3 * d.HT, G1 = 3 * d.D1T, G2 = 3 * NO;
        for (int l = 0; l < c->num_layers; ++l) {
            const LayerOff& lo = po.layer[l];
            const size_t t1 = lo.equi_b3, t2a = t1 + (size_t)nbw * G1 * 256, t2b = t2a + (size_t)nbr * G2 * 256;
            B3Jobs jb;
            jb.j[0] = B3Job{lo.dp0, d.WB, d.D1T, nbw, 0, t1, (size_t)3 * 256, (size_t)G1 * 256};
            jb.j[1] = B3Job{lo.rbfp, d.RB, NO, nbr, 0, t2a, (size_t)3 * 256, (size_t)G2 * 256};
            jb.j[2] = B3Job{lo.dp2, d.D1T, NO, nbd, 0, t2b, (size_t)3 * 256, (size_t)G2 * 256};
            jb.j[3] = B3Job{0, 0, 0, 0, 0, 0, 0, 0};
            const long long work = std::max<long long>((long long)d.D1T * nbw, (long long)NO * nbd) * 64;
            hipLaunchKernelGGL(k_pack_b3, dim3((unsigned)cdiv(work, 256), 3), dim3(256), 0, st, jb, (float*)packed);
        }
    }
    HIP_TRY(hipGetLastError());
    return OARD_OK;
}

void oard_topology_destroy(oard_topology* tp);

__global__ void k_spin(long long ticks) {
    const long long t0 = wall_clock64();
    while (wall_clock64() - t0 < ticks) __builtin_amdgcn_s_sleep(8);
}
static double spin_pair_us(hipStream_t a, hipStream_t b, bool both) {
    const long long ticks = 30000;
    (void)hipDeviceSynchronize();
    const auto t0 = std::chrono::steady_clock::now();
    hipLaunchKernelGGL(k_spin, dim3(1), dim3(64), 0, a, ticks);
    if (both) hipLaunchKernelGGL(k_spin, dim3(1), dim3(64), 0, b, ticks);
    (void)hipStreamSynchronize(a);
    if (both) (void)hipStreamSynchronize(b);
    return std::chrono::duration<double, std::micro>(std::chrono::steady_clock::now() - t0).count();
}
static bool streams_overlap(hipStream_t a, hipStream_t b, double one_us) { return spin_pair_us(a, b, true) < 1.6 * one_us; }
static hipStream_t* device_streams() {
    static hipStream_t all[64][3] = {};
    static std::mutex m;
    int d = 0;
    (void)hipGetDevice(&d);
    d &= 63;
    std::lock_guard<std::mutex> lk(m);
    if (!all[d][0]) {
        hipStream_t cand[8] = {};
        int n_cand = 0, taken = 0;
        for (; n_cand < 8; ++n_cand)
            if (hipStreamCreateWithFlags(&cand[n_cand], hipStreamNonBlocking) != hipSuccess) { (void)hipGetLastError(); break; }
        const bool calibrate = getenv("OARD_NO_STREAM_CALIBRATION") == nullptr;
        bool used[8] = {};
        double one_us = 0;
        if (calibrate && n_cand > 0) { (void)spin_pair_us(nullptr, nullptr, false); one_us = spin_pair_us(nullptr, nullptr, false); }
        for (int c = 0; c < n_cand && taken < 3 && calibrate; ++c) {
            bool ok = streams_overlap(nullptr, cand[c], one_us);
            for (int k = 0; k < taken && ok; ++k) ok = streams_overlap(all[d][k], cand[c], one_us);
            if (ok) { all[d][taken++] = cand[c]; used[c] = true; }
// ... 1148 lines not shown
           make_loss_cfg(c, norm_values, norm_biases, nullptr, pos_only, fixed_mask, T), t_int, gamma);
    HIP_TRY(hipGetLastError());
    return OARD_OK;
}
int oard_loss_terms(const oard_config* c, const oard_topology* topo, const float* const* eps, const float* const* net,
                    const float* const* z, const int64_t* const* one_hot, const int64_t* const* charge, const float* t_int,
                    const float* gamma, int T, const float* norm_values, const float* norm_biases, const float* scales, int pos_only,
                    int B, float* nll, float* terms, float* const* dnet, oard_stream_t stream) {
    topo_touch(topo, (hipStream_t)stream);
    if (!config_ok(c) || !topo || topo->n_parts != 1 || !eps || !net || !z || !one_hot || !charge || !t_int || !gamma || !nll || !terms ||
        !dnet || B < 1)
        return OARD_EINVAL;
    LossPtrs lp;
    memset(&lp, 0, sizeof(lp));
    for (int k = 0; k < c->n_obj; ++k) {
        if (c->node_nf[k] < 5 || c->node_nf[k] - 4 > 16) return OARD_EINVAL;
        lp.eps[k] = (float*)eps[k]; lp.net[k] = net[k]; lp.z[k] = (float*)z[k]; lp.one_hot[k] = (const long long*)one_hot[k];
        lp.charge[k] = (const long long*)charge[k]; lp.dnet[k] = dnet[k]; lp.node_nf[k] = c->node_nf[k];
    }
    const TopoDev& tp = topo->parts[0].d;
    LAUNCH(F_OTHER, k_loss_terms, tp.B, 64, (hipStream_t)stream, tp, lp, make_loss_cfg(c, norm_values, norm_biases, scales, pos_only, 0, T),
           t_int, gamma, B, nll, terms);
    HIP_TRY(hipGetLastError());
    return OARD_OK;
}
int oard_adamw_step(float* param, const float* grad, float* exp_avg, float* exp_avg_sq, float* max_exp_avg_sq, int64_t n, double lr,
                    double beta1, double beta2, double eps, double weight_decay, int64_t step, int amsgrad, double grad_scale,
                    oard_stream_t stream) {
    if (!param || !grad || !exp_avg || !exp_avg_sq || (amsgrad && !max_exp_avg_sq) || n < 0 || step < 1) return OARD_EINVAL;
    if (n == 0) return OARD_OK;
    const double bc1 = 1.0 - pow(beta1, (double)step), bc2 = 1.0 - pow(beta2, (double)step);
    LAUNCH(F_OTHER, k_adamw, cdiv(n, 256), 256, (hipStream_t)stream, param, grad, exp_avg, exp_avg_sq, max_exp_avg_sq, (long long)n,
           (float)(1.0 - lr * weight_decay), (float)(1.0 - beta1), (float)beta2, (float)(1.0 - beta2), (float)eps, (float)(lr / bc1),
           (float)(1.0 / sqrt(bc2)), amsgrad, (float)grad_scale);
    HIP_TRY(hipGetLastError());
    return OARD_OK;
}

int oard_adamw_step_dev(float* param, const float* grad, float* exp_avg, float* exp_avg_sq, float* max_exp_avg_sq, int64_t n, double lr,
                        double beta1, double beta2, double eps, double weight_decay, int amsgrad, int clip, double* clip_state,
                        int capacity, const float* grad_norm, const float* flag, float* out4, oard_stream_t stream) {
    if (!param || !grad || !exp_avg || !exp_avg_sq || (amsgrad && !max_exp_avg_sq) || n < 0 || !clip_state || capacity < 1 || capacity > 64 ||
        !grad_norm || !flag || !out4)
        return OARD_EINVAL;
    LAUNCH(F_OTHER, k_clip_decide, 1, 64, (hipStream_t)stream, clip_state, capacity, grad_norm, flag, clip, lr, beta1, beta2, eps, weight_decay, out4);
    if (n > 0)
        LAUNCH(F_OTHER, k_adamw_dev, cdiv(n, 256), 256, (hipStream_t)stream, param, grad, exp_avg, exp_avg_sq, max_exp_avg_sq, (long long)n, amsgrad,
               reinterpret_cast<const AdamScal*>(clip_state + 4 + capacity));
    HIP_TRY(hipGetLastError());
    return OARD_OK;
}

static bool ema_args_ok(const float* ema, double ema_decay) { return ema && ema_decay >= 0.0 && ema_decay <= 1.0; }

int oard_adamw_step_ema(float* param, const float* grad, float* exp_avg, float* exp_avg_sq, float* max_exp_avg_sq, int64_t n, double lr,
                        double beta1, double beta2, double eps, double weight_decay, int64_t step, int amsgrad, double grad_scale,
                        float* ema, double ema_decay, oard_stream_t stream) {
    if (!param || !grad || !exp_avg || !exp_avg_sq || (amsgrad && !max_exp_avg_sq) || n < 0 || step < 1 || !ema_args_ok(ema, ema_decay))
        return OARD_EINVAL;
    if (n == 0) return OARD_OK;
    const double bc1 = 1.0 - pow(beta1, (double)step), bc2 = 1.0 - pow(beta2, (double)step);
    LAUNCH(F_OTHER, k_adamw_ema, cdiv(n, 256), 256, (hipStream_t)stream, param, grad, exp_avg, exp_avg_sq, max_exp_avg_sq, (long long)n,
           (float)(1.0 - lr * weight_decay), (float)(1.0 - beta1), (float)beta2, (float)(1.0 - beta2), (float)eps, (float)(lr / bc1),
           (float)(1.0 / sqrt(bc2)), amsgrad, (float)grad_scale, ema, (float)ema_decay, (float)(1.0 - ema_decay));
    HIP_TRY(hipGetLastError());
    return OARD_OK;
}

int oard_adamw_step_dev_ema(float* param, const float* grad, float* exp_avg, float* exp_avg_sq, float* max_exp_avg_sq, int64_t n, double lr,
                            double beta1, double beta2, double eps, double weight_decay, int amsgrad, int clip, double* clip_state,
                            int capacity, const float* grad_norm, const float* flag, float* out4, float* ema, double ema_decay,
                            oard_stream_t stream) {
    if (!param || !grad || !exp_avg || !exp_avg_sq || (amsgrad && !max_exp_avg_sq) || n < 0 || !clip_state || capacity < 1 || capacity > 64 ||
        !grad_norm || !flag || !out4 || !ema_args_ok(ema, ema_decay))
        return OARD_EINVAL;
    LAUNCH(F_OTHER, k_clip_decide, 1, 64, (hipStream_t)stream, clip_state, capacity, grad_norm, flag, clip, lr, beta1, beta2, eps, weight_decay, out4);
    if (n > 0)
        LAUNCH(F_OTHER, k_adamw_dev_ema, cdiv(n, 256), 256, (hipStream_t)stream, param, grad, exp_avg, exp_avg_sq, max_exp_avg_sq, (long long)n,
               amsgrad, reinterpret_cast<const AdamScal*>(clip_state + 4 + capacity), ema, (float)ema_decay, (float)(1.0 - ema_decay));
    HIP_TRY(hipGetLastError());
    return OARD_OK;
}

int oard_ema_update(float* ema, const float* param, int64_t n, double ema_decay, oard_stream_t stream) {
    if (!param || n < 0 || !ema_args_ok(ema, ema_decay)) return OARD_EINVAL;
    if (n == 0) return OARD_OK;
    LAUNCH(F_OTHER, k_ema_update, cdiv(n, 256), 256, (hipStream_t)stream, ema, param, (long long)n, (float)ema_decay, (float)(1.0 - ema_decay));
    HIP_TRY(hipGetLastError());
    return OARD_OK;
}

int oard_train_scratch_entry(const oard_config* c, const oard_topology* topo, int which, size_t* offset_bytes, int64_t* rows,
                             int64_t* row_floats) {
    if (!config_ok(c) || !topo || topo->n_parts != 1 || !offset_bytes || !rows || !row_floats) return OARD_EINVAL;
    const TopoDev& d = topo->parts[0].d;
    const TrainWs w = make_train_ws(c, d);
    const RDims r(c->hidden, c->num_radial);
    switch (which) {
        case OARD_SCRATCH_XH: *offset_bytes = w.xh; *rows = d.N; *row_floats = r.HP; break;
        case OARD_SCRATCH_XQ: *offset_bytes = w.xq; *rows = d.N; *row_floats = 3 * r.HP; break;
        case OARD_SCRATCH_CR: *offset_bytes = w.cr; *rows = d.A + 1; *row_floats = 3 * r.HP; break;
        case OARD_SCRATCH_DCD: *offset_bytes = w.dcd; *rows = d.A + 1; *row_floats = 3 * r.HP; break;
        case OARD_SCRATCH_DCR: *offset_bytes = w.dcr; *rows = d.A + 1; *row_floats = 3 * r.HP; break;
        default: return OARD_EINVAL;
    }
    return OARD_OK;
}

int oard_tap(const oard_config* c, const oard_topology* topo, const void* ws_, int which, int layer, float* dst,
             oard_stream_t stream) {
    topo_touch(topo, (hipStream_t)stream);
    if (!config_ok(c) || !topo || !ws_ || !dst || layer != 0) return OARD_EINVAL;
    const RDims d(c->hidden, c->num_radial);
    ws_total(c, topo);
    hipStream_t st = (hipStream_t)stream;
    for (int p = 0; p < topo->n_parts; ++p) {
        const TopoDev& tp = topo->parts[p].d;
        const WsOff w = make_ws(c, tp);
        const char* ws = (const char*)ws_ + topo->parts[p].ws_off;
        auto nodes = [&](const float* src, int ld, int sections, int sect_pad, int sect_len) {
            const long long tot = (long long)tp.N * sections * sect_len;
            hipLaunchKernelGGL(k_tap_nodes, dim3((unsigned)cdiv(tot, 256)), dim3(256), 0, st, tp, src, ld, sections, sect_pad, sect_len, dst);
        };
        switch (which) {
            case OARD_TAP_S: nodes((const float*)(ws + w.s), d.HP, 1, d.HP, d.H); break;
            case OARD_TAP_VEC: nodes((const float*)(ws + topo->parts[p].vec_final), 3 * d.HP, 3, d.HP, d.H); break;
            case OARD_TAP_NE1: nodes((const float*)(ws + w.ne1), 3 * d.HP, 3, d.HP, d.H); break;
            case OARD_TAP_POS_FRAME: nodes((const float*)(ws + w.pf32), 3, 1, 3, 3); break;
            case OARD_TAP_DPOS: nodes((const float*)(ws + w.dpos), 3, 1, 3, 3); break;
            case OARD_TAP_HOUT: nodes((const float*)(ws + w.hout), 16, 1, 16, c->in_hidden); break;
            case OARD_TAP_LABELS:
                hipLaunchKernelGGL(k_tap_labels, dim3((unsigned)cdiv(tp.N, 256)), dim3(256), 0, st, tp, (const int*)(ws + w.labels), dst);
                break;
            case OARD_TAP_EDGE:
                if (tp.E > 0)
                    hipLaunchKernelGGL(k_tap_edges, dim3((unsigned)cdiv(tp.E * d.W, 256)), dim3(256), 0, st, tp,
                                       (const float*)(ws + w.ew), d.WP, d.W, dst);
                break;
            default: return OARD_EINVAL;
        }
    }
    HIP_TRY(hipGetLastError());
    return OARD_OK;
}

int oard_debug_stop_after(int code) { g_stop_after = code; return OARD_OK; }
int oard_debug_option(const char* name, int value) {
    if (!name) return OARD_EINVAL;
    static const struct { const char* name; int* value; } table[] = {
        {"gcl_variant", &g_fwd.gcl_variant}, {"equi_variant", &g_fwd.equi_variant}, {"node_variant", &g_fwd.node_variant},
        {"auto_small", &g_fwd.auto_small}, {"auto_tiny", &g_fwd.auto_tiny}, {"small_split", &g_fwd.small_split},
        {"gcl_persist", &g_fwd.gcl_persist}, {"gcl_grid", &g_fwd.gcl_grid}, {"gcl_skip", &g_fwd.gcl_skip}, {"equi_skip", &g_fwd.equi_skip},
        {"equi_l0_skip", &g_fwd.equi_l0_skip}, {"gcl_msum", &g_fwd.gcl_msum}, {"equi_rbf_table", &g_fwd.equi_rbf_table},
        {"skip_families", &g_skip_families}, {"parts", &g_parts}, {"sequential", &g_sequential}, {"poison", &g_poison}, {"npb", &g_npb},
        {"wgrad_wgs", &g_wgrad_wgs}, {"wgrad_t16", &g_wgrad_t16}, {"wgrad_queue", &g_wgrad_queue}, {"gate_fold", &g_gate_fold},
        {"wgrad_lds", &g_wgrad_lds}, {"wgrad_shapes", &g_wgrad_shapes}, {"train_dual", &g_train_dual}};
    if (strcmp(name, "experiments") == 0) return kV0 ? OARD_OK : OARD_EINVAL;
    if (strcmp(name, "gcl_msum_taken") == 0) return g_gcl_msum_taken ? OARD_OK : OARD_EINVAL;
    if (strcmp(name, "equi_rbf_taken") == 0) return g_equi_rbf_taken ? OARD_OK : OARD_EINVAL;
    if (strcmp(name, "equi_l0_taken") == 0) return g_equi_l0_taken ? OARD_OK : OARD_EINVAL;
    for (const auto& e : table) {
        if (strcmp(name, e.name) != 0) continue;
        if (!kV0 && value == 0 && strstr(name, "_variant")) return OARD_EINVAL;
        *e.value = e.value == &g_wgrad_shapes ? value & 3 : value;
        return OARD_OK;
    }
    return OARD_EINVAL;
}
#ifdef OARD_PHASE_PROBE
int oard_debug_probe_read(unsigned long long* out8) {
    if (!out8) return OARD_EINVAL;
    HIP_TRY(hipDeviceSynchronize());
    HIP_TRY(hipMemcpyFromSymbol(out8, HIP_SYMBOL(g_phase_probe), 8 * sizeof(unsigned long long)));
    unsigned long long z[8] = {};
    HIP_TRY(hipMemcpyToSymbol(HIP_SYMBOL(g_phase_probe), z, sizeof(z)));
    return OARD_OK;
}
#endif
#ifdef OARD_TIMELINE
int oard_debug_timeline_read(long long* out, int waves) {
    if (!out || waves < 1 || waves > 16) return OARD_EINVAL;
    HIP_TRY(hipDeviceSynchronize());
    HIP_TRY(hipMemcpyFromSymbol(out, HIP_SYMBOL(g_timeline), (size_t)waves * TL_MAX * sizeof(long long)));
    return OARD_OK;
}
#endif
#ifdef OARD_EXPERIMENTS
int oard_debug_fp_timeouts(unsigned int* out) {
    if (!out) return OARD_EINVAL;
    HIP_TRY(hipDeviceSynchronize());
    HIP_TRY(hipMemcpyFromSymbol(out, HIP_SYMBOL(g_fp_timeouts), sizeof(unsigned int)));
    return OARD_OK;
}
#endif
int oard_timing_enable(int on) { g_timing.on = on != 0; return OARD_OK; }
int oard_timing_reset(void) {
    g_timing.flush();
    for (int f = 0; f < F_COUNT; ++f) { g_timing.total_ms[f] = 0; g_timing.launches[f] = 0; }
    return OARD_OK;
}
int oard_timing_get(const char* family, double* total_ms, int64_t* launches) {
    if (!family || !total_ms || !launches) return OARD_EINVAL;
    g_timing.flush();
    for (int f = 0; f < F_COUNT; ++f)
        if (strcmp(family, kFamilyNames[f]) == 0) { *total_ms = g_timing.total_ms[f]; *launches = g_timing.launches[f]; return OARD_OK; }
    return OARD_EINVAL;
}

}
```

oareactdiff_amd/csrc/oard_kernels.h:

```cpp
#pragma once
#include "oard_engine.h"
#include "oard_layout.h"
#include "oard_rbf_table.h"

#define GEO_STRIDE 12
#define EPSF 1e-6

struct ColId {
    int lane, g, col;
    bool valid;
    long long c;
};
OARD_DEV ColId col_id(long long ncols, bool& wave_live) {
    ColId id;
    id.lane = threadIdx.x & 63;
    id.g = id.lane >> 4;
    const long long cb = (long long)blockIdx.x * 4 + (threadIdx.x >> 6);
    wave_live = cb * 16 < ncols;
    const long long c = cb * 16 + (id.lane & 15);
    id.valid = c < ncols;
    id.c = id.valid ? c : (ncols > 0 ? ncols - 1 : 0);
    id.col = (int)id.c;
    return id;
}

OARD_DEV int wave_max(int v) {
#pragma unroll
    for (int o = 1; o < 64; o <<= 1) v = max(v, __shfl_xor(v, o, 64));
    return v;
}

OARD_DEV f4 ld_f4(const float* p) { return *reinterpret_cast<const f4*>(p); }
OARD_DEV void st_f4(float* p, f4 v) { *reinterpret_cast<f4*>(p) = v; }

struct PackJob {
    const float* src;
    int src_ld, col_off;
    int msect_len, msect_pad, msects;
    int ksect_len, ksect_pad, ksects;
    int MT, KB;
    size_t dst;
    size_t tstride, bstride;
    int perm_ht;
    int transpose;
    int rows4;
    int tail_compact;
};

OARD_KERNEL __global__ void k_pack_matrix(PackJob j, float* __restrict__ blob) {
    const size_t total = (size_t)j.MT * j.KB * 256;
    for (size_t i = (size_t)blockIdx.x * blockDim.x + threadIdx.x; i < total; i += (size_t)gridDim.x * blockDim.x) {
        const int c = (int)(i & 3), lane = (int)((i >> 2) & 63);
        const size_t ch = i >> 8;
        const int b = (int)(ch % j.KB), t = (int)(ch / j.KB);
        const bool r4 = j.rows4 > 0 && t % j.rows4 == j.rows4 - 1;
        const bool tail = j.tail_compact && b == j.KB - 1 && !r4;
        const int r = 16 * t + (r4 ? (lane & 3) : (lane & 15)), k = tail ? 16 * b + (lane >> 4) : 16 * b + 4 * (lane >> 4) + c;
        const int rs = r / j.msect_pad, rw = r % j.msect_pad;
        const int ks = k / j.ksect_pad, kw = k % j.ksect_pad;
        float v = 0.f;
        if (rs < j.msects && rw < j.msect_len && ks < j.ksects && kw < j.ksect_len && !(tail && c != 0))
            v = j.transpose ? j.src[(size_t)(ks * j.ksect_len + kw) * j.src_ld + j.col_off + rs * j.msect_len + rw]
                            : j.src[(size_t)(rs * j.msect_len + rw) * j.src_ld + j.col_off + ks * j.ksect_len + kw];
        const int slot = j.perm_ht > 0 ? (t % j.perm_ht) * 3 + t / j.perm_ht : t;
        blob[j.dst + (size_t)slot * j.tstride + (size_t)b * j.bstride + (i & 255)] = v;
    }
}
OARD_KERNEL __global__ void k_pack_bias_chunks(const float* __restrict__ src, float* __restrict__ dst, int sect_len, int sect_pad,
                                   int sects, int n_tiles, size_t tstride, int perm_ht) {
    const int i = blockIdx.x * blockDim.x + threadIdx.x;
    if (i >= n_tiles * 256) return;
    const int t = i >> 8, lane = (i >> 2) & 63, c = i & 3;
    const int r = 16 * t + 4 * (lane >> 4) + c;
    const int s = r / sect_pad, w = r % sect_pad;
    const int slot = perm_ht > 0 ? (t % perm_ht) * 3 + t / perm_ht : t;
    dst[(size_t)slot * tstride + (i & 255)] = (src != nullptr && s < sects && w < sect_len) ? src[s * sect_len + w] : 0.f;
}
OARD_KERNEL __global__ void k_pack_vector(const float* __restrict__ src, float* __restrict__ dst, int sect_len, int sect_pad,
                              int sects, int n_dst) {
    const int i = blockIdx.x * blockDim.x + threadIdx.x;
    if (i >= n_dst) return;
    const int s = i / sect_pad, w = i % sect_pad;
    dst[i] = (src != nullptr && s < sects && w < sect_len) ? src[s * sect_len + w] : 0.f;
}
OARD_KERNEL __global__ void k_copy_raw(const float* __restrict__ src, float* __restrict__ dst, int n) {
    const int i = blockIdx.x * blockDim.x + threadIdx.x;
    if (i < n) dst[i] = src[i];
}
struct GenJob {
    int type;
    PackJob m;
    const float* src;
    size_t dst;
    int sect_len, sect_pad, sects, n;
    size_t tstride;
    int perm_ht;
    long long block0;
};
OARD_KERNEL __global__ __launch_bounds__(256) void k_pack_all(const GenJob* __restrict__ jobs, int n_jobs, float* __restrict__ blob) {
    int lo = 0, hi = n_jobs - 1;
    const long long b = blockIdx.x;
    while (lo < hi) {
        const int mid = (lo + hi + 1) >> 1;
        if (jobs[mid].block0 <= b) lo = mid; else hi = mid - 1;
    }
    const GenJob& J = jobs[lo];
    const size_t i = (size_t)(b - J.block0) * 256 + threadIdx.x;
    if (J.type == 0) {
        const PackJob& j = J.m;
        const size_t total = (size_t)j.MT * j.KB * 256;
        if (i >= total) return;
        const int c = (int)(i & 3), lane = (int)((i >> 2) & 63);
        const size_t ch = i >> 8;
        const int bb = (int)(ch % j.KB), t = (int)(ch / j.KB);
        const bool r4 = j.rows4 > 0 && t % j.rows4 == j.rows4 - 1;
        const bool tail = j.tail_compact && bb == j.KB - 1 && !r4;
        const int r = 16 * t + (r4 ? (lane & 3) : (lane & 15)), k = tail ? 16 * bb + (lane >> 4) : 16 * bb + 4 * (lane >> 4) + c;
        const int rs = r / j.msect_pad, rw = r % j.msect_pad;
        const int ks = k / j.ksect_pad, kw = k % j.ksect_pad;
        float v = 0.f;
        if (rs < j.msects && rw < j.msect_len && ks < j.ksects && kw < j.ksect_len && !(tail && c != 0))
            v = j.transpose ? j.src[(size_t)(ks * j.ksect_len + kw) * j.src_ld + j.col_off + rs * j.msect_len + rw]
                            : j.src[(size_t)(rs * j.msect_len + rw) * j.src_ld + j.col_off + ks * j.ksect_len + kw];
        const int slot = j.perm_ht > 0 ? (t % j.perm_ht) * 3 + t / j.perm_ht : t;
        blob[j.dst + (size_t)slot * j.tstride + (size_t)bb * j.bstride + (i & 255)] = v;
    } else if (J.type == 1) {
        if (i >= (size_t)J.n) return;
        const int s = (int)(i / J.sect_pad), w = (int)(i % J.sect_pad);
        blob[J.dst + i] = (J.src != nullptr && s < J.sects && w < J.sect_len) ? J.src[s * J.sect_len + w] : 0.f;
    } else if (J.type == 2) {
        if (i >= (size_t)J.n) return;
        const int t = (int)(i >> 8), lane = (int)((i >> 2) & 63), c = (int)(i & 3);
        const int r = 16 * t + 4 * (lane >> 4) + c;
        const int s = r / J.sect_pad, w = r % J.sect_pad;
        const int slot = J.perm_ht > 0 ? (t % J.perm_ht) * 3 + t / J.perm_ht : t;
        blob[J.dst + (size_t)slot * J.tstride + (i & 255)] = (J.src != nullptr && s < J.sects && w < J.sect_len) ? J.src[s * J.sect_len + w] : 0.f;
    } else {
        if (i < (size_t)J.n) blob[J.dst + i] = J.src[i];
    }
}

OARD_KERNEL __global__ void k_c0row(const float* __restrict__ lin3w0b , const float* __restrict__ lin3w2,
                        const float* __restrict__ lin3b2, const float* __restrict__ rl0b,
                        const float* __restrict__ rl2w, const float* __restrict__ rl2b, float* __restrict__ c0,
                        int H, int H4, int WP) {
    const int i = blockIdx.x * blockDim.x + threadIdx.x;
    if (i >= WP) return;
    float v = 0.f;
    if (i < 2 * H) {
        float a = lin3b2[0];
        for (int k = 0; k < H4; ++k) { const float x = lin3w0b[k]; a += lin3w2[k] * (x / (1.0f + expf(-x))); }
        v = a;
    } else if (i < 3 * H) {
        const int f = i - 2 * H;
        float a = rl2b[f];
        for (int k = 0; k < H; ++k) { const float x = rl0b[k]; a += rl2w[(size_t)f * H + k] * (x / (1.0f + expf(-x))); }
// ... 308 lines not shown
        if (a < tp.A) {
            const int i = tp.act_src[a], j = tp.act_tgt[a];
            const double rx = (double)pos[i * 3] - (double)pos[j * 3], ry = (double)pos[i * 3 + 1] - (double)pos[j * 3 + 1],
                         rz = (double)pos[i * 3 + 2] - (double)pos[j * 3 + 2];
            in = sqrt(rx * rx + ry * ry + rz * rz) < cutoff ? 1 : 0;
        }
        const int cnt = __syncthreads_count(in);
        if (threadIdx.x == 0) blk_cnt[blockIdx.x] = cnt;
    }
    if (a >= tp.A) return;
    const int i = tp.act_src[a], j = tp.act_tgt[a];
    const double rx = (double)pos[i * 3] - (double)pos[j * 3], ry = (double)pos[i * 3 + 1] - (double)pos[j * 3 + 1],
                 rz = (double)pos[i * 3 + 2] - (double)pos[j * 3 + 2];
    const double m = sqrt(rx * rx + ry * ry + rz * rz) < cutoff ? 1.0 : 0.0;
    const double ax = pf64[i * 3], ay = pf64[i * 3 + 1], az = pf64[i * 3 + 2];
    const double bx = pf64[j * 3], by = pf64[j * 3 + 1], bz = pf64[j * 3 + 2];
    const double dx = ax - bx, dy = ay - by, dz = az - bz;
    const double dist = sqrt(dx * dx + dy * dy + dz * dz);
    const double nr = dist + EPSF;
    double ux = dx / nr, uy = dy / nr, uz = dz / nr;
    double cx = ay * bz - az * by, cy = az * bx - ax * bz, cz = ax * by - ay * bx;
    const double cn = sqrt(cx * cx + cy * cy + cz * cz) + EPSF;
    cx /= cn; cy /= cn; cz /= cn;
    double vx = uy * cz - uz * cy, vy = uz * cx - ux * cz, vz = ux * cy - uy * cx;
    const double d = dist * m;
    const double env = 0.5 * (cos(d * M_PI / cutoff) + 1.0);
    float* g = geo + a * GEO_STRIDE;
    g[0] = (float)d; g[1] = (float)env;
    g[2] = (float)(ux * m); g[3] = (float)(uy * m); g[4] = (float)(uz * m);
    g[5] = (float)(cx * m); g[6] = (float)(cy * m); g[7] = (float)(cz * m);
    g[8] = (float)(vx * m); g[9] = (float)(vy * m); g[10] = (float)(vz * m);
    g[11] = (float)m;
    d64[a] = d;
}

__device__ inline void lin3u_f64(const float* __restrict__ p, double x, double& f, double& df) {
    double h[48], dh[48];
    for (int k = 0; k < 48; ++k) {
        const double w = (double)p[3 * k], z = w * x + (double)p[144 + k], s = 1.0 / (1.0 + exp(-z));
        h[k] = z * s; dh[k] = w * s * (1.0 + z * (1.0 - s));
    }
    f = (double)p[592]; df = 0.0;
    for (int j = 0; j < 8; ++j) {
        double z = (double)p[576 + j], dz = 0.0;
        for (int k = 0; k < 48; ++k) { const double w = (double)p[192 + j * 48 + k]; z += w * h[k]; dz += w * dh[k]; }
        const double s = 1.0 / (1.0 + exp(-z));
        f += (double)p[584 + j] * z * s; df += (double)p[584 + j] * dz * s * (1.0 + z * (1.0 - s));
    }
}
OARD_DEV float lin3u_table_eval(const float* __restrict__ tab, float x) {
    const float u = x * (1.0f / L3T_H), fl = floorf(u), t = u - fl;
    const int i = (int)fl + L3T_N / 2;
    const float f0 = tab[2 * i], d0 = tab[2 * i + 1], f1 = tab[2 * i + 2], d1 = tab[2 * i + 3];
    const float t2 = t * t, t3 = t2 * t;
    return (2.f * t3 - 3.f * t2 + 1.f) * f0 + (t3 - 2.f * t2 + t) * d0 + (3.f * t2 - 2.f * t3) * f1 + (t3 - t2) * d1;
}
struct L3tJobs { size_t l3u[OARD_MAX_LAYERS], l3t[OARD_MAX_LAYERS]; };
OARD_KERNEL __global__ __launch_bounds__(256) void k_lin3u_table_fill(float* __restrict__ blob, L3tJobs j) {
    const float* p = blob + j.l3u[blockIdx.y];
    float* tab = blob + j.l3t[blockIdx.y];
    const int i = blockIdx.x * 256 + threadIdx.x;
    double f, df;
    lin3u_f64(p, ((double)i - L3T_N / 2) * (double)L3T_H, f, df);
    tab[2 * i] = (float)f; tab[2 * i + 1] = (float)(df * (double)L3T_H);
    if (i == 0) {
        lin3u_f64(p, (double)L3T_X, f, df);
        tab[2 * L3T_N] = (float)f; tab[2 * L3T_N + 1] = (float)(df * (double)L3T_H);
        tab[2 * (L3T_N + 1)] = 0.f; tab[2 * (L3T_N + 1) + 1] = 0.f; tab[2 * (L3T_N + 1) + 2] = 0.f; tab[2 * (L3T_N + 1) + 3] = 0.f;
    }
}
OARD_KERNEL __global__ __launch_bounds__(256) void k_lin3u_table_check(float* __restrict__ blob, L3tJobs j) {
    __shared__ float red_e[256], red_f[256];
    const float* p = blob + j.l3u[blockIdx.y];
    float* tab = blob + j.l3t[blockIdx.y];
    const int i = blockIdx.x * 256 + threadIdx.x, t = threadIdx.x;
    const double x = ((double)i - L3T_N / 2 + 0.5) * (double)L3T_H;
    double f, df;
    lin3u_f64(p, x, f, df);
    red_e[t] = fabsf(lin3u_table_eval(tab, (float)x) - (float)f);
    red_f[t] = fmaxf(fabsf(tab[2 * i]), fabsf((float)f));
    __syncthreads();
    for (int d = 128; d >= 1; d >>= 1) {
        if (t < d) { red_e[t] = fmaxf(red_e[t], red_e[t + d]); red_f[t] = fmaxf(red_f[t], red_f[t + d]); }
        __syncthreads();
    }
    if (t == 0) {
        unsigned* u = reinterpret_cast<unsigned*>(tab + 2 * (L3T_N + 1));
        atomicMax(u + 1, __float_as_uint(red_e[0]));
        atomicMax(u + 2, __float_as_uint(red_f[0]));
        __threadfence();
        if (atomicAdd(u + 3, 1u) == gridDim.x - 1) {
            __threadfence();
            const float e = __uint_as_float(atomicMax(u + 1, 0u)), fm = __uint_as_float(atomicMax(u + 2, 0u));
            tab[2 * (L3T_N + 1)] = (e <= 2e-7f * fmaxf(fm, 1e-30f) && fm < 3e38f) ? 1.0f : 0.0f;
        }
    }
}
struct RbtJobs { size_t w[OARD_MAX_LAYERS], tab[OARD_MAX_LAYERS], flag[OARD_MAX_LAYERS]; size_t means, betas; int H, HT, R; };
OARD_KERNEL __global__ __launch_bounds__(256) void k_rbf_table_fill(float* __restrict__ blob, RbtJobs j) {
    const long long id = (long long)blockIdx.x * 256 + threadIdx.x;
    if (id >= (long long)3 * j.HT * (RBT_N + 1) * 4) return;
    const int l = blockIdx.y, g = (int)(id & 3), pt = (int)((id >> 2) % (RBT_N + 1)), slot = (int)((id >> 2) / (RBT_N + 1));
    const int tt = slot / 3, th = slot - 3 * tt;
    float* out = blob + j.tab[l] + ((size_t)slot * (RBT_N + 1) + pt) * 32 + 8 * g;
    const double u = (double)pt * (1.0 / RBT_N);
    for (int s = 0; s < 4; ++s) {
        const int feat = 16 * tt + 4 * g + s;
        float f32 = 0.f, d32 = 0.f;
        if (feat < j.H) {
            double f, df;
            rbt_eval_f64(blob + j.w[l] + (size_t)(th * j.H + feat) * j.R, blob + j.means, blob + j.betas, j.R, u, f, df);
            rbt_entry(f, df, f32, d32);
        }
        out[s] = f32; out[4 + s] = d32;
    }
    if (id == 0) { float* fl = blob + j.flag[l]; fl[0] = 0.f; fl[1] = 0.f; fl[2] = 0.f; fl[3] = 0.f; }
}
OARD_KERNEL __global__ __launch_bounds__(256) void k_rbf_table_check(float* __restrict__ blob, RbtJobs j) {
    __shared__ double red_e[4][256], red_f[4][256];
    const int l = blockIdx.y, slot = blockIdx.x >> 2, g = blockIdx.x & 3, t = threadIdx.x;
    const int tt = slot / 3, th = slot - 3 * tt;
    const float* tab = blob + j.tab[l] + (size_t)slot * (RBT_N + 1) * 32 + 8 * g;
    for (int s = 0; s < 4; ++s) {
        const int feat = 16 * tt + 4 * g + s;
        double e = 0.0, fm = 0.0;
        if (feat < j.H)
            for (int i = t; i < RBT_N; i += 256) {
                const float* p0 = tab + (size_t)i * 32 + s;
                double f, df;
                rbt_eval_f64(blob + j.w[l] + (size_t)(th * j.H + feat) * j.R, blob + j.means, blob + j.betas, j.R, ((double)i + 0.5) * (1.0 / RBT_N), f, df);
                const double dev = fabs(rbt_midpoint(p0[0], p0[4], p0[32], p0[36]) - f);
                e = dev > e || dev != dev ? dev : e;
                fm = fmax(fm, fmax(fabs((double)p0[0]), fabs(f)));
            }
        red_e[s][t] = e; red_f[s][t] = fm;
    }
    __syncthreads();
    if (t == 0) {
        bool ok = true;
        for (int s = 0; s < 4; ++s) {
            double e = 0.0, fm = 0.0;
            for (int k = 0; k < 256; ++k) { e = red_e[s][k] > e || red_e[s][k] != red_e[s][k] ? red_e[s][k] : e; fm = fmax(fm, red_f[s][k]); }
            ok = ok && (16 * tt + 4 * g + s >= j.H || rbt_channel_ok(e, fm));
        }
        unsigned* u = reinterpret_cast<unsigned*>(blob + j.flag[l]);
        if (!ok) atomicAdd(u + 1, 1u);
        __threadfence();
        if (atomicAdd(u + 2, 1u) == gridDim.x - 1) {
            __threadfence();
            blob[j.flag[l]] = atomicAdd(u + 1, 0u) == 0u ? 1.0f : 0.0f;
        }
    }
}
struct ZeroRows { float* p[64]; int n[64]; int count; };
OARD_KERNEL __global__ __launch_bounds__(256) void k_zero_rows(ZeroRows z) {
    if ((int)blockIdx.x >= z.count) return;
    float* p = z.p[blockIdx.x];
    for (int i = threadIdx.x; i < z.n[blockIdx.x]; i += 256) p[i] = 0.f;
}
OARD_KERNEL __global__ __launch_bounds__(256) void k_active_list(TopoDev tp, const float* __restrict__ geo, const int* __restrict__ blk_cnt,
                                                     int* __restrict__ rows, int* __restrict__ src, int* __restrict__ pre, int* __restrict__ n_act) {
    __shared__ int red[256];
    __shared__ int wsum[4];
    int base = 0;
    for (int b = threadIdx.x; b < (int)blockIdx.x; b += 256) base += blk_cnt[b];
    red[threadIdx.x] = base;
    __syncthreads();
    for (int d = 128; d >= 1; d >>= 1) {
        if ((int)threadIdx.x < d) red[threadIdx.x] += red[threadIdx.x + d];
        __syncthreads();
    }
    base = red[0];
    const long long a = (long long)blockIdx.x * 256 + threadIdx.x;
    const bool on = a < tp.A && geo[a * GEO_STRIDE + 11] > 0.f;
    const unsigned long long bal = __ballot(on);
    const int lane = threadIdx.x & 63, wave = threadIdx.x >> 6;
    const int in_wave = __popcll(bal & ((1ull << lane) - 1ull));
    if (lane == 0) wsum[wave] = __popcll(bal);
    __syncthreads();
    int off = base + in_wave;
    for (int w = 0; w < wave; ++w) off += wsum[w];
    if (a < tp.A) pre[a] = off;
    if (on) { rows[off] = (int)a; src[off] = tp.act_src[a]; }
    if (a == tp.A - 1) { const int tot = off + (on ? 1 : 0); pre[tp.A] = tot; *n_act = tot; }
}
OARD_KERNEL __global__ void k_rbf(TopoDev tp, const double* __restrict__ d64, const float* __restrict__ geo,
                      const float* __restrict__ means, const float* __restrict__ betas, double cutoff,
                      float* __restrict__ rbuf, float* __restrict__ ew, int R, int RP, int H, int WP, float* __restrict__ rbt = nullptr) {
    const long long i = (long long)blockIdx.x * blockDim.x + threadIdx.x;
    if (i >= tp.A * RP) return;
    const long long a = i / RP;
    const int k = (int)(i % RP);
    float v = 0.f;
    if (k < R) {
        const double d = d64[a], m = (double)geo[a * GEO_STRIDE + 11];
        if (rbt != nullptr && k == 1) {
            const RbtAt at = rbt_locate(d, cutoff, m);
            float w[4];
            rbt_weights(at, w);
            float* r = rbt + a * RBT_ROW;
            st_f4(r, (f4){__int_as_float(at.idx), w[0], w[1], w[2]});
            st_f4(r + 4, (f4){w[3], 0.f, 0.f, 0.f});
        }
        double rb = 0.5 * (cos(d * M_PI / cutoff) + 1.0);
        rb = d < cutoff ? rb : 0.0;
        const double q = exp(-d) - (double)means[k];
        v = (float)(rb * exp(-(double)betas[k] * q * q) * m);
        ew[(size_t)a * WP + 3 * H + k] = v;
        if (k == 0)
            for (int c = 3 * H + R; c < WP; ++c) ew[(size_t)a * WP + c] = 0.f;
    }
    rbuf[i] = v;
}

OARD_KERNEL __global__ void k_fill_edges(const float* __restrict__ c0, float* __restrict__ ew, long long E, int WP) {
    const int per = WP / 4;
    const long long total = E * per;
    for (long long i = (long long)blockIdx.x * blockDim.x + threadIdx.x; i < total; i += (long long)gridDim.x * blockDim.x)
        st_f4(ew + i * 4, ld_f4(c0 + (i % per) * 4));
}

template <class D>
__global__ __launch_bounds__(256) void k_node_embed(TopoDev tp, const float* __restrict__ wb, PackOff po,
                                                    const float* __restrict__ hin, float* __restrict__ zemb,
                                                    float* __restrict__ nb) {
    bool live; const ColId id = col_id(tp.N, live);
    if (!live) return;
    f4 in[1] = {ld_blk(hin, id.c, 16, 0, id.lane)};
    f4 v[D::HT];
#pragma unroll
    for (int t = 0; t < D::HT; ++t) {
        f4 z = dense_tile<1>(wb + po.emb, t, in, id.lane, ld_vec(wb + po.emb_b, t, id.lane));
        if (id.valid) st_blk(zemb, id.c, D::HP, t, id.lane, z);
        v[t] = dense_tile<1>(wb + po.nbemb, t, in, id.lane, ld_vec(wb + po.nbemb_b, t, id.lane));
    }
    layer_norm<D::HT, D::H, false>(v, nullptr, nullptr, id.lane);
    if (id.valid)
#pragma unroll
        for (int t = 0; t < D::HT; ++t) st_blk(nb, id.c, D::HP, t, id.lane, v[t]);
}

template <class D>
__global__ __launch_bounds__(256) void k_radial_lin(TopoDev tp, const float* __restrict__ wb, PackOff po,
                                                    const float* __restrict__ rbuf, const float* __restrict__ geo,
                                                    float* __restrict__ ew) {
    bool live; const ColId id = col_id(tp.A, live);
    if (!live) return;
    f4 rb[D::RB];
#pragma unroll
    for (int b = 0; b < D::RB; ++b) rb[b] = ld_blk(rbuf, id.c, D::RP, b, id.lane);
    f4 h1[D::HT];
    dense_regs<D::RB, D::HT, true, true>(wb + po.rl0, wb + po.rl0_b, rb, h1, id.lane);
    const float env = geo[id.c * GEO_STRIDE + 1];
    const size_t row = (size_t)id.c * D::WP + 2 * D::H;
#pragma unroll
    for (int t = 0; t < D::HT; ++t) {
        f4 f = dense_tile<D::HT>(wb + po.rl2, t, h1, id.lane, ld_vec(wb + po.rl2_b, t, id.lane));
        if (id.valid && 16 * t + 4 * id.g < D::H) st_f4(ew + row + 16 * t + 4 * id.g, f * env);
    }
}

template <class D>
__global__ __launch_bounds__(256) void k_neighbor(TopoDev tp, const float* __restrict__ wb, PackOff po,
                                                  const float* __restrict__ zemb, const float* __restrict__ nb,
                                                  const float* __restrict__ ew, float* __restrict__ s,
                                                  float* __restrict__ s1) {
    bool live; const ColId id = col_id(tp.N, live);
    if (!live) return;
    const int n = id.col, smp = tp.node_sample[n], s0 = tp.sample_ptr[smp], ns = tp.sample_ptr[smp + 1] - s0;
    f4 acc[D::HT];
#pragma unroll
    for (int t = 0; t < D::HT; ++t) acc[t] = f4zero();
    const int mx = wave_max(ns);
    for (int k = 0; k < mx; ++k) {
        const int m = s0 + k;
        if (k < ns && m != n) {
            const int r = tp.edge_row[tp.edge_ptr[m] + (n - s0) - (n > m ? 1 : 0)];
            const float* frow = (r < tp.A ? ew + (size_t)r * D::WP : wb + po.c0row) + 2 * D::H;
#pragma unroll
            for (int t = 0; t < D::HT; ++t)
                if (16 * t + 4 * id.g < D::H)
                    acc[t] += ld_f4(frow + 16 * t + 4 * id.g) * ld_blk(nb, m, D::HP, t, id.lane);
        }
    }
#pragma unroll
    for (int t = 0; t < D::HT; ++t) acc[t] += ld_blk(zemb, n, D::HP, t, id.lane);
    if (id.valid)
#pragma unroll
        for (int t = 0; t < D::HT; ++t) st_blk(s, n, D::HP, t, id.lane, acc[t]);
    f4 y[D::HT];
    dense_regs<D::HT, D::HT, false, true>(wb + po.s2v, wb + po.s2v_b, acc, y, id.lane);
    layer_norm<D::HT, D::H, false>(y, nullptr, nullptr, id.lane);
    if (id.valid)
#pragma unroll
        for (int t = 0; t < D::HT; ++t) st_blk(s1, n, D::HP, t, id.lane, silu4(y[t]));
}

template <class D>
__global__ __launch_bounds__(256) void k_s2v_agg(TopoDev tp, const float* __restrict__ s1, const float* __restrict__ ew,
                                                 const float* __restrict__ geo, float* __restrict__ ne1) {
    bool live; const ColId id = col_id(tp.N, live);
    if (!live) return;
    const int n = id.col, a0 = tp.act_ptr[n], cnt = tp.act_ptr[n + 1] - a0;
    const int mx = wave_max(cnt);
    const bool fok = true;
    for (int t = 0; t < D::HT; ++t) {
// ... 423 lines not shown
```

oareactdiff_amd/csrc/oard_layout.h:

```cpp
#pragma once
#include <hip/hip_runtime.h>
#include <stdint.h>
#include <stddef.h>
#include "../../include/oard.h"

#define OARD_MAX_LAYERS 16
#define OARD_MAX_GROUP 1024

template <int H_, int R_>
struct Dims {
    static constexpr int H = H_, R = R_;
    static constexpr int HT = (H + 15) / 16, HP = HT * 16;
    static constexpr int W = 3 * H + R, WB = (W + 15) / 16, WP = WB * 16;
    static constexpr int RB = (R + 15) / 16, RP = RB * 16;
    static constexpr int H2 = H / 2, PB = (H2 + 15) / 16, PP = PB * 16;
    static constexpr int D1T = (3 * H + 15) / 16, D1P = D1T * 16;
    static constexpr int H4 = H / 4;
    static_assert(H % 4 == 0 && R % 4 == 0, "feature widths must be multiples of 4");
};

struct RDims {
    int H, R, HT, HP, W, WB, WP, RB, RP, H2, PB, PP, D1T, D1P, H4;
    explicit RDims(int h, int r) {
        H = h; R = r; HT = (H + 15) / 16; HP = HT * 16; W = 3 * H + R; WB = (W + 15) / 16; WP = WB * 16;
        RB = (R + 15) / 16; RP = RB * 16; H2 = H / 2; PB = (H2 + 15) / 16; PP = PB * 16;
        D1T = (3 * H + 15) / 16; D1P = D1T * 16; H4 = H / 4;
    }
};

#define L3T_X 16.0f
#define L3T_H 0.03125f
#define L3T_N 1024
#define L3T_FLOATS (2 * (L3T_N + 1) + 4)

struct LayerOff {
    size_t ln_g_w, ln_g_b, W1a, b1, W1b, W1c, W2, b2, watt, batt, W3, b3, nm0, nm0b, nm1, nm1b;
    size_t ln_q_w, ln_q_b, xp0, xp2, dp0, dp0b, dp2, dp2b, rbfp;
    size_t rbfw, rbff, rbft;
    size_t vp, xv0, xv2, l3u;
    size_t l3t;
    size_t gcl_stream, equi_stream;
    size_t gcl_b3, equi_b3;
    int xcross;
};
struct PackOff {
    size_t emb, emb_b, nbemb, nbemb_b, s2v, s2v_b, rl0, rl0_b, rl2, rl2_b;
    size_t lin3;
    size_t pe0;
    size_t pe1, embout, embout_b, v1p, v2p, un0, un0_b, un2, un2_b;
    size_t c0row;
    size_t u0;
    size_t rbf_means, rbf_betas;
    size_t enc[OARD_MAX_OBJECTS], dec[OARD_MAX_OBJECTS];
    LayerOff layer[OARD_MAX_LAYERS];
    size_t head;
    size_t total;
    int signed_scal;
};

struct TopoDev {
    int N, B, n_obj, n_groups;
    int npb;
    long long E, A;
    const int *node_obj, *node_row, *node_ref, *node_tidx, *node_sample, *sample_ptr;
    const int *edge_ptr, *edge_src, *edge_tgt;
    const int *edge_row;
    const int *row_src, *row_tgt;
    const int *row_eid;
    const int *grp_ptr;
    const int *act_ptr, *act_src, *act_tgt, *act_edge;
    const long long *ref_edge_ptr;
    long long CI, CX;
    const int *col_info;
    const int *node_cols;
};

struct ActList {
    const int* rows;
    const int* src;
    const int* pre;
    const int* n;
};

#define OARD_MAX_PARTS 8
struct TopoPart {
    TopoDev d;
    void* dev_block = nullptr;
    size_t dev_cap = 0;
    void* stage = nullptr;
    size_t stage_cap = 0;
    size_t ws_off = 0;
    int conc = 1;
    mutable size_t vec_final = 0;
};
struct oard_topology {
    int device = 0;
    int n_parts = 0;
    TopoPart parts[OARD_MAX_PARTS];
    int n_obj = 0, B = 0;
    long long N = 0, E = 0, A = 0;
    int max_group = 0, max_ns = 0;
    int obj_start[OARD_MAX_OBJECTS + 1] = {};
    hipStream_t side[OARD_MAX_PARTS] = {};
    hipEvent_t ev_fork = nullptr, ev_join[OARD_MAX_PARTS] = {};
    void* ref_block = nullptr;
    size_t ref_cap = 0;
    void* ref_stage = nullptr;
    size_t ref_stage_cap = 0;
    hipEvent_t ready = nullptr;
    mutable hipStream_t used_on[4] = {};
    mutable int n_used = 0;
    mutable bool used_many = false;
    const int *ref_sample = nullptr, *ref_rank = nullptr;
    const long long* ref_ptr = nullptr;
    int N_ref = 0;
};

struct WsOff {
    size_t pos, pf64, pf32, x1, pp0, labels, hin, zemb, nb, s, s1, ne1, xh, P, Q, xq, vec, vec2, v2buf, sc0, vdot,
        geo, d64, rbuf, ew, mbuf, xmsg, vmsg, dpos, hout, total;
    size_t al_rows, al_src, al_pre, al_cnt, al_n;
    size_t rbt;
    size_t d1s;
    size_t small_a;
};
```

oareactdiff_amd/csrc/oard_plan.h:

```cpp
#pragma once
#include <algorithm>
#include "../../include/oard.h"

struct FwdOptions {
    int gcl_variant = 2;
    int equi_variant = 2;
    int node_variant = 1;
    int auto_small = 4;
    int auto_tiny = 8;
    int small_split = 128;
    int gcl_persist = 1;
    int gcl_grid = 0;
    int gcl_skip = 1;
    int equi_skip = 1;
    int equi_l0_skip = 1;
    int gcl_msum = 1;
    int equi_rbf_table = 1;
};

enum GclShape {
    GCL_INVALID = 0,
    GCL_V0,
    GCL_PERSIST, GCL_RING3,
    GCL_W4, GCL_SMALL, GCL_B3,
    GCL_TRAIN_PERSIST, GCL_TRAIN_RING3, GCL_TRAIN_B3,
    GCL_X0 = 100
};
enum EquiShape { EQ_INVALID = 0, EQ_V0, EQ_W8, EQ_W4, EQ_SMALL, EQ_SMALL_SPLIT, EQ_B3, EQ_TRAIN, EQ_TRAIN_B3 };
enum NodeForm { NODE_V0 = 0, NODE_ROWS, NODE_LARGE };

struct GclLaunch { long long r0, r1; bool s1, s3; GclShape shape; long long grid; };
struct GclLayer { int n; GclLaunch l[2]; };
struct FwdPlanIn {
    FwdOptions opt;
    int precision;
    bool train;
    int conc, npb, cus;
    long long A, E, CI, CX;
    int num_layers;
    bool scratch;
    unsigned rbf_good = 0;
};
struct FwdPlan {
    int num_layers;
    bool fill_edges;
    bool init_v1;
    bool scalarize_tiles;
    bool msum;
    GclLayer gcl[4];
    EquiShape equi;
    bool use_al;
    NodeForm node;
    bool l0_skip;
    bool rbf_table[16];
    const GclLayer& gcl_at(int l) const { return gcl[(l == 0 ? 1 : 0) | (l == num_layers - 1 ? 2 : 0)]; }
};

inline long long plan_cdiv(long long a, long long b) { return (a + b - 1) / b; }
inline int plan_demote(const FwdPlanIn& in, int v, long long n, long long small_tiles, int w4, int lat) {
    const long long load = plan_cdiv(n, 16) * in.conc;
    if (v == 2 && load <= small_tiles * in.opt.auto_small) v = w4;
    if ((v == 2 || v == w4) && load <= 512LL * in.opt.auto_tiny) v = lat;
    return v;
}
inline GclShape plan_gcl_shape(const FwdPlanIn& in, long long n) {
    const int persist = in.opt.gcl_persist;
    if (in.train) return (in.precision & OARD_PREC_TRAIN_BF16X3) ? GCL_TRAIN_B3 : persist ? GCL_TRAIN_PERSIST : GCL_TRAIN_RING3;
    const int v = plan_demote(in, in.opt.gcl_variant, n, 1024, 3, 6);
    switch (v) {
        case 0: return GCL_V0;
        case 2: return (in.precision & OARD_PREC_GCL_BF16X3) ? GCL_B3 : (persist > 1 || (persist == 1 && in.conc == 1)) ? GCL_PERSIST : GCL_RING3;
        case 3: return GCL_W4;
        case 6: return GCL_SMALL;
#ifdef OARD_EXPERIMENTS
        case 4: case 5: case 7: case 8: case 9: case 10: case 11: case 12: return GclShape(GCL_X0 + v);
#endif
        default: return GCL_INVALID;
    }
}
inline long long plan_gcl_grid(const FwdPlanIn& in, GclShape s, long long n) {
    if (s == GCL_PERSIST || s == GCL_TRAIN_PERSIST) {
        const long long nhalf = plan_cdiv(plan_cdiv(n, 16), 4), g = in.opt.gcl_grid;
        return std::min(nhalf, g > 0 ? g : g < 0 ? plan_cdiv(nhalf, 2 * -g) : in.conc > 1 ? std::max(1, in.cus / 2) : in.cus);
    }
    return plan_cdiv(n, s == GCL_SMALL ? 16 : (s == GCL_V0 || s == GCL_W4 || s == GCL_X0 + 12) ? 64 : (s == GCL_X0 + 10 || s == GCL_X0 + 11) ? 192 : 128);
}
inline EquiShape plan_equi_shape(const FwdPlanIn& in) {
    if (in.train) return (in.precision & OARD_PREC_TRAIN_BF16X3) ? EQ_TRAIN_B3 : EQ_TRAIN;
    switch (plan_demote(in, in.opt.equi_variant, in.A, 512, 1, 4)) {
        case 0: return EQ_V0;
        case 1: return EQ_W4;
        case 2: return (in.precision & OARD_PREC_EQUI_BF16X3) ? EQ_B3 : EQ_W8;
        case 4: return in.scratch && plan_cdiv(in.A, 16) * in.conc <= in.opt.small_split ? EQ_SMALL_SPLIT : EQ_SMALL;
        default: return EQ_INVALID;
    }
}
inline bool plan_rbf_wanted(const FwdPlanIn& in) {
    return !in.train && in.opt.equi_rbf_table && in.A > 0 && plan_equi_shape(in) == EQ_W8;
}
inline FwdPlan make_fwd_plan(FwdPlanIn in) {
    if (in.train) { in.opt.gcl_variant = in.opt.equi_variant = 2; in.opt.node_variant = 1; in.opt.gcl_skip = 1; }
    const FwdOptions& o = in.opt;
    const bool nv1 = o.node_variant == 1 && o.equi_variant != 0, skip = o.gcl_skip && o.gcl_variant != 0;
    FwdPlan p = {};
    p.num_layers = in.num_layers;
    p.fill_edges = !skip;
    p.init_v1 = o.node_variant >= 1;
    p.scalarize_tiles = plan_cdiv(in.A, 64) * in.conc <= 2048;
    p.node = !nv1 ? NODE_V0 : in.npb <= 4 ? NODE_ROWS : NODE_LARGE;
    p.equi = plan_equi_shape(in);
    p.use_al = !in.train && o.equi_skip && in.A > 0 && nv1;
    p.l0_skip = !in.train && o.equi_l0_skip && in.A > 0 && p.node == NODE_LARGE && p.equi == EQ_W8;
    for (int l = 0; l < 16; ++l)
        p.rbf_table[l] = !in.train && o.equi_rbf_table && in.A > 0 && p.equi == EQ_W8 && l < in.num_layers && ((in.rbf_good >> l) & 1u);
    auto throughput = [&](long long n) { const GclShape s = plan_gcl_shape(in, n); return n == 0 || s == GCL_PERSIST || s == GCL_RING3; };
    p.msum = !in.train && o.gcl_msum && in.E > 0 && o.gcl_variant == 2 && p.node == NODE_LARGE && throughput(in.CI) && throughput(in.CX);
    const long long inner = p.msum ? in.CI : in.A, all = p.msum ? in.CI + in.CX : in.E;
    for (int k = 0; k < 4; ++k) {
        GclLayer& g = p.gcl[k];
        auto add = [&](long long r0, long long r1, bool s1, bool s3) {
            const GclShape s = plan_gcl_shape(in, r1 - r0);
            if (r1 > r0) g.l[g.n++] = GclLaunch{r0, r1, s1, s3, s, plan_gcl_grid(in, s, r1 - r0)};
        };
        const bool s1 = !(skip && (k & 1)), s3 = !(skip && (k & 2));
        if (s1 && s3) add(0, all, true, true);
        else { add(0, inner, true, true); add(inner, all, s1, s3); }
    }
    return p;
}
```

Baseline: 3761 reaction-steps/s.

## Replace per-edge radial MLP with a precomputed Hermite distance lookup table

Adds a distance-indexed cubic Hermite table holding the radial MLP output and its derivative per hidden channel. The table is built and accuracy-checked once per weight blob, and on by default. The forward pass then interpolates the table per edge in a fused k_rbf_dist kernel instead of running the k_radial_lin matrix multiply over all edges. This removes per-edge GEMM work and a kernel launch, at the cost of an interpolation approximation error, extra blob memory, and a one-time build with a host sync.

```diff
diff --git a/oareactdiff_amd/_capi.py b/oareactdiff_amd/_capi.py
--- a/oareactdiff_amd/_capi.py
+++ b/oareactdiff_amd/_capi.py
@@ -162,7 +162,7 @@
     L.oard_timing_reset.argtypes = []; L.oard_timing_reset.restype = C.c_int
     L.oard_timing_get.argtypes = [C.c_char_p, C.POINTER(C.c_double), C.POINTER(i64)]; L.oard_timing_get.restype = C.c_int
     for env, opt in (("OARD_GCL_VARIANT", b"gcl_variant"), ("OARD_EQUI_VARIANT", b"equi_variant"),
-                     ("OARD_NODE_VARIANT", b"node_variant"), ("OARD_GCL_SKIP", b"gcl_skip"), ("OARD_EQUI_SKIP", b"equi_skip"), ("OARD_EQUI_L0_SKIP", b"equi_l0_skip"), ("OARD_EQUI_RBF_TABLE", b"equi_rbf_table"),("OARD_GCL_MSUM", b"gcl_msum"), ("OARD_GCL_PERSIST", b"gcl_persist"), ("OARD_GCL_GRID", b"gcl_grid"), ("OARD_PARTS", b"parts"), ("OARD_SEQUENTIAL", b"sequential"), ("OARD_POISON", b"poison"), ("OARD_AUTO_SMALL", b"auto_small"), ("OARD_AUTO_TINY", b"auto_tiny"), ("OARD_NPB", b"npb"),
+                     ("OARD_NODE_VARIANT", b"node_variant"), ("OARD_GCL_SKIP", b"gcl_skip"), ("OARD_EQUI_SKIP", b"equi_skip"), ("OARD_EQUI_L0_SKIP", b"equi_l0_skip"), ("OARD_EQUI_RBF_TABLE", b"equi_rbf_table"), ("OARD_RADIAL_TABLE", b"radial_table"),("OARD_GCL_MSUM", b"gcl_msum"), ("OARD_GCL_PERSIST", b"gcl_persist"), ("OARD_GCL_GRID", b"gcl_grid"), ("OARD_PARTS", b"parts"), ("OARD_SEQUENTIAL", b"sequential"), ("OARD_POISON", b"poison"), ("OARD_AUTO_SMALL", b"auto_small"), ("OARD_AUTO_TINY", b"auto_tiny"), ("OARD_NPB", b"npb"),
                      ("OARD_WGRAD_WGS", b"wgrad_wgs"), ("OARD_WGRAD_LDS", b"wgrad_lds"), ("OARD_WGRAD_T16", b"wgrad_t16"), ("OARD_WGRAD_QUEUE", b"wgrad_queue"), ("OARD_GATE_FOLD", b"gate_fold"), ("OARD_WGRAD_SHAPES", b"wgrad_shapes"), ("OARD_TRAIN_DUAL", b"train_dual"), ("OARD_SMALL_SPLIT", b"small_split"),
                      ("OARD_SKIP_FAMILIES", b"skip_families")):
         if os.environ.get(env) not in (None, ""):
diff --git a/oareactdiff_amd/build.py b/oareactdiff_amd/build.py
--- a/oareactdiff_amd/build.py
+++ b/oareactdiff_amd/build.py
@@ -6,7 +6,7 @@
 
 CSRC = os.path.join(os.path.dirname(os.path.abspath(__file__)), "csrc")
 LIB = os.environ.get("OARD_LIB") or os.path.join(CSRC, "liboard_hip.so")
-_EDGE = ["oard_engine.h", "oard_layout.h", "oard_rbf_table.h", "oard_kernels.h", "oard_edge_v1.h", "oard_inst.h"]
+_EDGE = ["oard_engine.h", "oard_layout.h", "oard_rbf_table.h", "oard_dist_table.h", "oard_kernels.h", "oard_edge_v1.h", "oard_inst.h"]
 SOURCES = {
     "oard_hip.hip": None,
     "oard_general.hip": ["oard_general.h"],
diff --git a/oareactdiff_amd/csrc/oard_dist_table.h b/oareactdiff_amd/csrc/oard_dist_table.h
--- /dev/null
+++ b/oareactdiff_amd/csrc/oard_dist_table.h
@@ -0,0 +1,98 @@
+#pragma once
+#include "oard_rbf_table.h"
+
+#ifndef DT_NU
+#define DT_NU 2048
+#define DT_J0 64
+#define DT_PER_A 64
+#endif
+
+struct DtGrid { int nu, nd, points; double d0, cutoff; };
+RBT_HD DtGrid dt_grid(double cutoff) {
+    DtGrid g;
+    g.nu = DT_NU - DT_J0;
+    g.d0 = -log((double)DT_J0 / (double)DT_NU);
+    const double span = (cutoff - g.d0) * (double)DT_PER_A;
+    g.nd = span > 1.0 ? (span < 1048576.0 ? (int)ceil(span) : 1048576) : 1;
+    g.points = g.nu + 1 + g.nd + 1 + 2;
+    g.cutoff = cutoff;
+    return g;
+}
+RBT_HD int dt_pseudo(const DtGrid& g) { return g.nu + g.nd + 2; }
+RBT_HD size_t dt_point_floats(int HT) { return (size_t)HT * 32; }
+RBT_HD size_t dt_table_floats(const DtGrid& g, int HT) { return (size_t)g.points * dt_point_floats(HT); }
+RBT_HD size_t dt_flag_floats(int HT) { return 4 + (size_t)HT * 16 * 4; }
+
+struct DtPoint { double d, slope; bool masked; };
+RBT_HD DtPoint dt_point(const DtGrid& g, int p, int half) {
+    DtPoint r;
+    r.masked = p >= dt_pseudo(g);
+    if (r.masked) { r.d = 0.0; r.slope = 0.0; }
+    else if (p <= g.nu) {
+        const double u = ((double)(DT_J0 + p) + 0.5 * half) / (double)DT_NU;
+        r.d = -log(u); r.slope = -1.0 / (u * (double)DT_NU);
+    } else { r.d = g.d0 + ((double)(p - g.nu - 1) + 0.5 * half) / (double)DT_PER_A; r.slope = 1.0 / (double)DT_PER_A; }
+    return r;
+}
+RBT_HD bool dt_is_interval(const DtGrid& g, int p) { return p >= 0 && p != g.nu && p != g.nu + 1 + g.nd && p <= dt_pseudo(g); }
+
+RBT_HD void dt_env(double d, double cutoff, bool masked, double& rb, double& drb) {
+    const double a = 3.14159265358979323846 / cutoff;
+    rb = masked ? 1.0 : 0.5 * (cos(d * a) + 1.0);
+    drb = masked ? 0.0 : -0.5 * a * sin(d * a);
+}
+RBT_HD void dt_emb(double d, double rb, double drb, bool masked, double mean, double beta, double& e, double& de) {
+    const double u = exp(-d), q = u - mean, g = exp(-beta * q * q);
+    e = masked ? 0.0 : rb * g;
+    de = masked ? 0.0 : drb * g + rb * g * (2.0 * beta * q * u);
+}
+RBT_HD void dt_silu(double z, double dz, double& h, double& dh) {
+    const double s = 1.0 / (1.0 + exp(-z));
+    h = z * s; dh = dz * s * (1.0 + z * (1.0 - s));
+}
+struct DtWeights { const float *w1, *b1, *w2, *b2, *means, *betas; int H, R; };
+RBT_HD void dt_hidden(const DtWeights& w, const DtPoint& pt, double cutoff, double* h, double* dh, double* e, double* de) {
+    double rb, drb;
+    dt_env(pt.d, cutoff, pt.masked, rb, drb);
+    for (int k = 0; k < w.R; ++k) dt_emb(pt.d, rb, drb, pt.masked, (double)w.means[k], (double)w.betas[k], e[k], de[k]);
+    for (int c = 0; c < w.H; ++c) {
+        double z = (double)w.b1[c], dz = 0.0;
+        for (int k = 0; k < w.R; ++k) { z += (double)w.w1[(size_t)c * w.R + k] * e[k]; dz += (double)w.w1[(size_t)c * w.R + k] * de[k]; }
+        dt_silu(z, dz, h[c], dh[c]);
+    }
+}
+RBT_HD void dt_channel(const DtWeights& w, const DtPoint& pt, double cutoff, const double* h, const double* dh, int c, double& f, double& df) {
+    double rb, drb, y = (double)w.b2[c], dy = 0.0;
+    dt_env(pt.d, cutoff, pt.masked, rb, drb);
+    for (int j = 0; j < w.H; ++j) { y += (double)w.w2[(size_t)c * w.H + j] * h[j]; dy += (double)w.w2[(size_t)c * w.H + j] * dh[j]; }
+    f = rb * y; df = drb * y + rb * dy;
+}
+RBT_HD void dt_entry(double f, double df, const DtPoint& pt, float& fo, float& dfo) { fo = (float)f; dfo = (float)(df * pt.slope); }
+
+struct DtAt { int idx; double frac, factor; };
+RBT_HD DtAt dt_locate(const DtGrid& g, double d, double mask) {
+    DtAt r;
+    r.factor = 1.0;
+    if (!(mask > 0.0) || !(d < g.cutoff)) {
+        r.idx = dt_pseudo(g); r.frac = 0.0;
+        if (mask > 0.0) r.factor = 0.5 * (cos(d * 3.14159265358979323846 / g.cutoff) + 1.0);
+        return r;
+    }
+    const double x = exp(-d) * (double)DT_NU;
+    if (x >= (double)DT_J0) {
+        int i = (int)floor(x);
+        i = i > DT_NU - 1 ? DT_NU - 1 : i;
+        r.idx = i - DT_J0; r.frac = x - (double)i;
+    } else {
+        const double y = (d - g.d0) * (double)DT_PER_A;
+        int i = (int)floor(y);
+        i = i < 0 ? 0 : (i > g.nd - 1 ? g.nd - 1 : i);
+        r.idx = g.nu + 1 + i; r.frac = y - (double)i;
+    }
+    return r;
+}
+RBT_HD void dt_weights(const DtAt& at, float (&w)[4]) {
+    double h[4];
+    rbt_basis(at.frac, h);
+    for (int j = 0; j < 4; ++j) w[j] = (float)(h[j] * at.factor);
+}
diff --git a/oareactdiff_amd/csrc/oard_hip.hip b/oareactdiff_amd/csrc/oard_hip.hip
--- a/oareactdiff_amd/csrc/oard_hip.hip
+++ b/oareactdiff_amd/csrc/oard_hip.hip
@@ -69,6 +69,7 @@
 int g_gcl_msum_taken = 0;
 int g_equi_l0_taken = 0;
 int g_equi_rbf_taken = 0;
+int g_radial_table_taken = 0;
 int g_parts = 0;
 int g_wgrad_shapes = 3;
 int g_wgrad_t16 = 256;
@@ -146,6 +147,7 @@
     po.c0row = take(d.WP);
     po.u0 = take(d.HP);
     po.rbf_means = take(d.RP); po.rbf_betas = take(d.RP);
+    po.rlw = take((size_t)d.H * d.R + d.H + (size_t)d.H * d.H + d.H);
     for (int k = 0; k < c->n_obj; ++k) {
         const int dd = c->node_nf[k] - 3;
         po.enc[k] = take((size_t)2 * dd * dd + 2 * dd + (size_t)emb * 2 * dd + emb);
@@ -184,6 +186,7 @@
     }
     po.head = cur;
     for (int l = 0; l < c->num_layers; ++l) po.layer[l].rbft = take(rbt_layer_floats(d.HT));
+    po.dtt = take(dt_table_floats(dt_grid((double)c->cutoff), d.HT)); po.dtf = take(dt_flag_floats(d.HT));
     po.total = cur;
     po.signed_scal = c->reflect_equiv ? 0 : 1;
     for (int l = 0; l < c->num_layers; ++l) po.layer[l].xcross = c->reflect_equiv ? 0 : 1;
@@ -283,38 +286,61 @@
         return OARD_OK;
     }
 };
-struct RbfTablesOf { const void* blob; unsigned good; };
+struct RbfTablesOf { const void* blob; unsigned built, good, dist_good; };
 static std::mutex g_rbf_mu;
 static std::vector<RbfTablesOf> g_rbf_known;
 static void rbf_tables_forget(const void* blob) {
     std::lock_guard<std::mutex> lk(g_rbf_mu);
     g_rbf_known.erase(std::remove_if(g_rbf_known.begin(), g_rbf_known.end(), [&](const RbfTablesOf& e) { return e.blob == blob; }), g_rbf_known.end());
 }
-static int rbf_tables_for(const oard_config* c, const PackOff& po, const float* blob, hipStream_t st, unsigned* good) {
-    *good = 0;
+static int rbf_tables_for(const oard_config* c, const PackOff& po, const float* blob, hipStream_t st, bool want_rbf, bool want_dist,
+                          unsigned* good, unsigned* dist_good) {
+    *good = 0; *dist_good = 0;
+    const unsigned want = (want_rbf ? 1u : 0u) | (want_dist ? 2u : 0u);
     std::lock_guard<std::mutex> lk(g_rbf_mu);
-    for (const RbfTablesOf& e : g_rbf_known) if (e.blob == blob) { *good = e.good; return OARD_OK; }
+    RbfTablesOf known{blob, 0, 0, 0};
+    for (const RbfTablesOf& e : g_rbf_known) if (e.blob == blob) known = e;
+    auto answer = [&]() { if (want_rbf) *good = known.good; if (want_dist) *dist_good = known.dist_good; };
+    const unsigned todo = want & ~known.built;
+    if (todo == 0) { answer(); return OARD_OK; }
     hipStreamCaptureStatus cap = hipStreamCaptureStatusNone;
     HIP_TRY(hipStreamIsCapturing(st, &cap));
-    if (cap != hipStreamCaptureStatusNone) return OARD_OK;
+    if (cap != hipStreamCaptureStatusNone) { answer(); return OARD_OK; }
     const RDims d(c->hidden, c->num_radial);
-    RbtJobs j;
-    memset(&j, 0, sizeof(j));
-    for (int l = 0; l < c->num_layers; ++l) { j.w[l] = po.layer[l].rbfw; j.tab[l] = po.layer[l].rbft; j.flag[l] = po.layer[l].rbff; }
-    j.means = po.rbf_means; j.betas = po.rbf_betas; j.H = d.H; j.HT = d.HT; j.R = d.R;
-    hipLaunchKernelGGL(k_rbf_table_fill, dim3((unsigned)cdiv((long long)3 * d.HT * (RBT_N + 1) * 4, 256), (unsigned)c->num_layers), dim3(256), 0, st,
-                       const_cast<float*>(blob), j);
-    hipLaunchKernelGGL(k_rbf_table_check, dim3((unsigned)(3 * d.HT * 4), (unsigned)c->num_layers), dim3(256), 0, st, const_cast<float*>(blob), j);
-    HIP_TRY(hipGetLastError());
     std::vector<float> flags((size_t)c->num_layers, 0.f);
-    for (int l = 0; l < c->num_layers; ++l)
-        HIP_TRY(hipMemcpyAsync(&flags[l], blob + po.layer[l].rbff, sizeof(float), hipMemcpyDeviceToHost, st));
+    float dist_flag = 0.f;
+    if (todo & 1u) {
+        RbtJobs j;
+        memset(&j, 0, sizeof(j));
+        for (int l = 0; l < c->num_layers; ++l) { j.w[l] = po.layer[l].rbfw; j.tab[l] = po.layer[l].rbft; j.flag[l] = po.layer[l].rbff; }
+        j.means = po.rbf_means; j.betas = po.rbf_betas; j.H = d.H; j.HT = d.HT; j.R = d.R;
+        hipLaunchKernelGGL(k_rbf_table_fill, dim3((unsigned)cdiv((long long)3 * d.HT * (RBT_N + 1) * 4, 256), (unsigned)c->num_layers), dim3(256), 0, st,
+                           const_cast<float*>(blob), j);
+        hipLaunchKernelGGL(k_rbf_table_check, dim3((unsigned)(3 * d.HT * 4), (unsigned)c->num_layers), dim3(256), 0, st, const_cast<float*>(blob), j);
+        HIP_TRY(hipGetLastError());
+        for (int l = 0; l < c->num_layers; ++l)
+            HIP_TRY(hipMemcpyAsync(&flags[l], blob + po.layer[l].rbff, sizeof(float), hipMemcpyDeviceToHost, st));
+    }
+    const bool dist_fits = d.H <= DT_MAX_W && d.R <= DT_MAX_W;
+    if ((todo & 2u) && dist_fits) {
+        DtJobs j;
+        memset(&j, 0, sizeof(j));
+        j.w1 = po.rlw; j.b1 = j.w1 + (size_t)d.H * d.R; j.w2 = j.b1 + d.H; j.b2 = j.w2 + (size_t)d.H * d.H;
+        j.means = po.rbf_means; j.betas = po.rbf_betas; j.tab = po.dtt; j.flag = po.dtf; j.H = d.H; j.HT = d.HT; j.R = d.R;
+        j.g = dt_grid((double)c->cutoff);
+        hipLaunchKernelGGL(k_dist_table_fill, dim3((unsigned)j.g.points), dim3(256), 0, st, const_cast<float*>(blob), j);
+        hipLaunchKernelGGL(k_dist_table_check, dim3((unsigned)(dt_pseudo(j.g) + 1)), dim3(256), 0, st, const_cast<float*>(blob), j);
+        HIP_TRY(hipGetLastError());
+        HIP_TRY(hipMemcpyAsync(&dist_flag, blob + po.dtf, sizeof(float), hipMemcpyDeviceToHost, st));
+    }
     HIP_TRY(hipStreamSynchronize(st));
-    unsigned mask = 0;
-    for (int l = 0; l < c->num_layers; ++l) if (flags[l] == 1.0f) mask |= 1u << l;
+    if (todo & 1u) for (int l = 0; l < c->num_layers; ++l) if (flags[l] == 1.0f) known.good |= 1u << l;
+    if ((todo & 2u) && dist_flag == 1.0f) known.dist_good = 1u;
+    known.built |= todo;
+    g_rbf_known.erase(std::remove_if(g_rbf_known.begin(), g_rbf_known.end(), [&](const RbfTablesOf& e) { return e.blob == blob; }), g_rbf_known.end());
     if (g_rbf_known.size() >= 64) g_rbf_known.erase(g_rbf_known.begin());
-    g_rbf_known.push_back({blob, mask});
-    *good = mask;
+    g_rbf_known.push_back(known);
+    answer();
     return OARD_OK;
 }
 
@@ -528,8 +554,12 @@
     const unsigned gN = (unsigned)cdiv(N, 64), gA = (unsigned)cdiv(A, 64);
     const double cutoff = (double)c->cutoff;
     FwdPlanIn plan_in{opt, c->precision, train, topo->conc, tp.npb, device_cus(), A, E, tp.CI, tp.CX, c->num_layers, w.small_a != 0};
-    if (plan_rbf_wanted(plan_in)) { const int rc = rbf_tables_for(c, po, wb, st, &plan_in.rbf_good); if (rc != OARD_OK) return rc; }
+    if (plan_rbf_wanted(plan_in) || plan_dist_wanted(plan_in)) {
+        const int rc = rbf_tables_for(c, po, wb, st, plan_rbf_wanted(plan_in), plan_dist_wanted(plan_in), &plan_in.rbf_good, &plan_in.dist_good);
+        if (rc != OARD_OK) return rc;
+    }
     const FwdPlan plan = make_fwd_plan(plan_in);
+    g_radial_table_taken = plan.radial_table;
     bool any_rbt = false, all_rbt = c->num_layers > 0;
     for (int l = 0; l < c->num_layers; ++l) { any_rbt = any_rbt || plan.rbf_table[l]; all_rbt = all_rbt && plan.rbf_table[l]; }
     g_equi_rbf_taken = all_rbt;
@@ -548,11 +578,15 @@
     if (A > 0) {
         LAUNCH(F_INIT, k_edge_geo, cdiv(A, 256), 256, st, tp, (const float*)pos, (const double*)pf64, cutoff, geo, d64, use_al ? al_cnt : nullptr);
         if (use_al) LAUNCH(F_INIT, k_active_list, cdiv(A, 256), 256, st, tp, (const float*)geo, (const int*)al_cnt, (int*)al.rows, (int*)al.src, (int*)al.pre, (int*)al.n);
-        LAUNCH(F_INIT, k_rbf, cdiv(A * D::RP, 256), 256, st, tp, (const double*)d64, (const float*)geo,
+        if (plan.radial_table)
+            LAUNCH(F_INIT, (k_rbf_dist<D>), cdiv(A * D::RP, 256), 256, st, tp, (const double*)d64, (const float*)geo, wb + po.rbf_means, wb + po.rbf_betas,
+                   cutoff, dt_grid(cutoff), wb + po.dtt, all_rbt ? (float*)nullptr : rbuf, ew, any_rbt ? (float*)(ws + w.rbt) : (float*)nullptr);
+        else LAUNCH(F_INIT, k_rbf, cdiv(A * D::RP, 256), 256, st, tp, (const double*)d64, (const float*)geo,
                wb + po.rbf_means, wb + po.rbf_betas, cutoff, rbuf, ew, D::R, D::RP, D::H, D::WP, any_rbt ? (float*)(ws + w.rbt) : (float*)nullptr);
     }
     LAUNCH(F_INIT, (k_node_embed<D>), gN, 256, st, tp, wb, po, (const float*)hin, zemb, nb);
-    if (A > 0) LAUNCH(F_INIT, (k_radial_lin<D>), gA, 256, st, tp, wb, po, (const float*)rbuf, (const float*)geo, ew);
+    if (A > 0 && !plan.radial_table)
+        LAUNCH(F_INIT, (k_radial_lin<D>), gA, 256, st, tp, wb, po, (const float*)rbuf, (const float*)geo, ew);
     constexpr int NW = D::HT <= 16 ? D::HT : 8;
     const unsigned gNb = (unsigned)cdiv(N, tp.npb);
     if (plan.init_v1) {
@@ -827,6 +861,8 @@
     pk.nat(pi.pe1_w, d.H2, 0, H, d.H2, d.HT, d.PB, po.pe1);
     pk.nat(pi.embout_w, H, 0, C, H, 1, d.HT, po.embout);    pk.vec(pi.embout_b, C, 16, 1, 16, po.embout_b);
     pk.raw(pi.means, R, po.rbf_means);                      pk.raw(pi.betas, R, po.rbf_betas);
+    pk.raw(pi.rl0_w, H * R, po.rlw);                        pk.raw(pi.rl0_b, H, po.rlw + (size_t)H * R);
+    pk.raw(pi.rl2_w, H * H, po.rlw + (size_t)H * R + H);    pk.raw(pi.rl2_b, H, po.rlw + (size_t)H * R + H + (size_t)H * H);
     const int o = pi.out0;
     pk.nat(o + 0, H, 0, H, H, d.HT, d.HT, po.v1p);
     pk.vec(o + 1, H, d.HP, 1, d.HP, po.v2p);
@@ -2281,12 +2317,14 @@
         {"auto_small", &g_fwd.auto_small}, {"auto_tiny", &g_fwd.auto_tiny}, {"small_split", &g_fwd.small_split},
         {"gcl_persist", &g_fwd.gcl_persist}, {"gcl_grid", &g_fwd.gcl_grid}, {"gcl_skip", &g_fwd.gcl_skip}, {"equi_skip", &g_fwd.equi_skip},
         {"equi_l0_skip", &g_fwd.equi_l0_skip}, {"gcl_msum", &g_fwd.gcl_msum}, {"equi_rbf_table", &g_fwd.equi_rbf_table},
+        {"radial_table", &g_fwd.radial_table},
         {"skip_families", &g_skip_families}, {"parts", &g_parts}, {"sequential", &g_sequential}, {"poison", &g_poison}, {"npb", &g_npb},
         {"wgrad_wgs", &g_wgrad_wgs}, {"wgrad_t16", &g_wgrad_t16}, {"wgrad_queue", &g_wgrad_queue}, {"gate_fold", &g_gate_fold},
         {"wgrad_lds", &g_wgrad_lds}, {"wgrad_shapes", &g_wgrad_shapes}, {"train_dual", &g_train_dual}};
     if (strcmp(name, "experiments") == 0) return kV0 ? OARD_OK : OARD_EINVAL;
     if (strcmp(name, "gcl_msum_taken") == 0) return g_gcl_msum_taken ? OARD_OK : OARD_EINVAL;
     if (strcmp(name, "equi_rbf_taken") == 0) return g_equi_rbf_taken ? OARD_OK : OARD_EINVAL;
+    if (strcmp(name, "radial_table_taken") == 0) return g_radial_table_taken ? OARD_OK : OARD_EINVAL;
     if (strcmp(name, "equi_l0_taken") == 0) return g_equi_l0_taken ? OARD_OK : OARD_EINVAL;
     for (const auto& e : table) {
         if (strcmp(name, e.name) != 0) continue;
diff --git a/oareactdiff_amd/csrc/oard_kernels.h b/oareactdiff_amd/csrc/oard_kernels.h
--- a/oareactdiff_amd/csrc/oard_kernels.h
+++ b/oareactdiff_amd/csrc/oard_kernels.h
@@ -2,6 +2,7 @@
 #include "oard_engine.h"
 #include "oard_layout.h"
 #include "oard_rbf_table.h"
+#include "oard_dist_table.h"
 
 #define GEO_STRIDE 12
 #define EPSF 1e-6
@@ -616,6 +617,135 @@
         }
     }
 }
+#define DT_MAX_W 256
+struct DtJobs { size_t w1, b1, w2, b2, means, betas, tab, flag; int H, HT, R; DtGrid g; };
+__device__ inline void dt_hidden_wg(const float* __restrict__ blob, const DtJobs& j, const DtPoint& pt, double* e, double* de, double* h, double* dh) {
+    const int t = threadIdx.x;
+    double rb, drb;
+    dt_env(pt.d, j.g.cutoff, pt.masked, rb, drb);
+    for (int k = t; k < j.R; k += 256) dt_emb(pt.d, rb, drb, pt.masked, (double)blob[j.means + k], (double)blob[j.betas + k], e[k], de[k]);
+    __syncthreads();
+    for (int c = t; c < j.H; c += 256) {
+        const float* w = blob + j.w1 + (size_t)c * j.R;
+        double z = (double)blob[j.b1 + c], dz = 0.0;
+        for (int k = 0; k < j.R; ++k) { z += (double)w[k] * e[k]; dz += (double)w[k] * de[k]; }
+        dt_silu(z, dz, h[c], dh[c]);
+    }
+    __syncthreads();
+}
+OARD_KERNEL __global__ __launch_bounds__(256) void k_dist_table_fill(float* __restrict__ blob, DtJobs j) {
+    __shared__ double e[DT_MAX_W], de[DT_MAX_W], h[DT_MAX_W], dh[DT_MAX_W];
+    const int p = blockIdx.x, t = threadIdx.x;
+    const DtPoint pt = dt_point(j.g, p, 0);
+    dt_hidden_wg(blob, j, pt, e, de, h, dh);
+    const DtWeights w{blob + j.w1, blob + j.b1, blob + j.w2, blob + j.b2, blob + j.means, blob + j.betas, j.H, j.R};
+    float* out = blob + j.tab + (size_t)p * dt_point_floats(j.HT);
+    for (int c = t; c < j.HT * 16; c += 256) {
+        float f32 = 0.f, d32 = 0.f;
+        if (c < j.H) {
+            double f, df;
+            dt_channel(w, pt, j.g.cutoff, h, dh, c, f, df);
+            dt_entry(f, df, pt, f32, d32);
+        }
+        out[(c >> 2) * 8 + (c & 3)] = f32; out[(c >> 2) * 8 + 4 + (c & 3)] = d32;
+    }
+    if (p == 0) for (int i = t; i < (int)dt_flag_floats(j.HT); i += 256) blob[j.flag + i] = 0.f;
+}
+OARD_KERNEL __global__ __launch_bounds__(256) void k_dist_table_check(float* __restrict__ blob, DtJobs j) {
+    __shared__ double e[DT_MAX_W], de[DT_MAX_W], h[DT_MAX_W], dh[DT_MAX_W];
+    __shared__ int last, bad[256];
+    const int p = blockIdx.x, t = threadIdx.x;
+    unsigned long long* red = reinterpret_cast<unsigned long long*>(blob + j.flag + 4);
+    unsigned* u = reinterpret_cast<unsigned*>(blob + j.flag);
+    if (dt_is_interval(j.g, p)) {
+        const DtPoint pt = dt_point(j.g, p, 1);
+        dt_hidden_wg(blob, j, pt, e, de, h, dh);
+        const DtWeights w{blob + j.w1, blob + j.b1, blob + j.w2, blob + j.b2, blob + j.means, blob + j.betas, j.H, j.R};
+        const float* p0 = blob + j.tab + (size_t)p * dt_point_floats(j.HT);
+        const float* p1 = p0 + dt_point_floats(j.HT);
+        for (int c = t; c < j.H; c += 256) {
+            double f, df;
+            dt_channel(w, pt, j.g.cutoff, h, dh, c, f, df);
+            const int o = (c >> 2) * 8 + (c & 3);
+            const double dev = fabs(rbt_midpoint(p0[o], p0[o + 4], p1[o], p1[o + 4]) - f);
+            atomicMax(red + 2 * c, (unsigned long long)__double_as_longlong(dev));
+            atomicMax(red + 2 * c + 1, (unsigned long long)__double_as_longlong(fmax(fabs((double)p0[o]), fabs(f))));
+        }
+    }
+    __threadfence();
+    __syncthreads();
+    if (t == 0) last = atomicAdd(u + 2, 1u) == gridDim.x - 1 ? 1 : 0;
+    __syncthreads();
+    if (!last) return;
+    __threadfence();
+    int nbad = 0;
+    for (int c = t; c < j.H; c += 256) {
+        const double dev = __longlong_as_double((long long)atomicMax(red + 2 * c, 0ull)), fm = __longlong_as_double((long long)atomicMax(red + 2 * c + 1, 0ull));
+        nbad += rbt_channel_ok(dev, fm) ? 0 : 1;
+    }
+    bad[t] = nbad;
+    __syncthreads();
+    if (t == 0) {
+        int n = 0;
+        for (int k = 0; k < 256; ++k) n += bad[k];
+        blob[j.flag] = n == 0 ? 1.0f : 0.0f;
+    }
+}
+template <class D>
+__global__ __launch_bounds__(256) void k_rbf_dist(TopoDev tp, const double* __restrict__ d64, const float* __restrict__ geo,
+                                                  const float* __restrict__ means, const float* __restrict__ betas, double cutoff, DtGrid dtg,
+                                                  const float* __restrict__ tab, float* __restrict__ rbuf, float* __restrict__ ew,
+                                                  float* __restrict__ rbt) {
+    constexpr int RP = D::RP, ROWS = 256 / RP + 2;
+    static_assert(RP <= 256, "a row's threads fit one workgroup");
+    __shared__ double s_rb[ROWS], s_u[ROWS], s_m[ROWS];
+    __shared__ float s_w[ROWS][4];
+    __shared__ int s_idx[ROWS];
+    const long long i0 = (long long)blockIdx.x * 256, i = i0 + threadIdx.x, a0 = i0 / RP;
+    if ((int)threadIdx.x < ROWS && a0 + threadIdx.x < tp.A) {
+        const long long a = a0 + threadIdx.x;
+        const double d = d64[a], m = (double)geo[a * GEO_STRIDE + 11];
+        if (rbt != nullptr && a * RP + 1 >= i0 && a * RP + 1 < i0 + 256) {
+            const RbtAt at = rbt_locate(d, cutoff, m);
+            float w[4];
+            rbt_weights(at, w);
+            float* r = rbt + a * RBT_ROW;
+            st_f4(r, (f4){__int_as_float(at.idx), w[0], w[1], w[2]});
+            st_f4(r + 4, (f4){w[3], 0.f, 0.f, 0.f});
+        }
+        double rb = 0.5 * (cos(d * M_PI / cutoff) + 1.0);
+        rb = d < cutoff ? rb : 0.0;
+        s_rb[threadIdx.x] = rb; s_u[threadIdx.x] = exp(-d); s_m[threadIdx.x] = m;
+        const DtAt at = dt_locate(dtg, d, m);
+        dt_weights(at, s_w[threadIdx.x]);
+        s_idx[threadIdx.x] = min(max(at.idx, 0), dt_pseudo(dtg));
+    }
+    __syncthreads();
+    if (i >= tp.A * RP) return;
+    const long long a = i / RP;
+    const int k = (int)(i % RP), r = (int)(a - a0);
+    float v = 0.f;
+    if (k < D::R) {
+        const double q = s_u[r] - (double)means[k];
+        v = (float)(s_rb[r] * exp(-(double)betas[k] * q * q) * s_m[r]);
+        ew[(size_t)a * D::WP + 3 * D::H + k] = v;
+        if (k == 0)
+            for (int c = 3 * D::H + D::R; c < D::WP; ++c) ew[(size_t)a * D::WP + c] = 0.f;
+    }
+    if (rbuf != nullptr) rbuf[i] = v;
+    const float w0 = s_w[r][0], w1 = s_w[r][1], w2 = s_w[r][2], w3 = s_w[r][3];
+    for (int q = k; q < D::H / 4; q += RP) {
+        const float* p0 = tab + (size_t)s_idx[r] * (D::HT * 32) + q * 8;
+        const float* p1 = p0 + D::HT * 32;
+        const f4 f0 = ld_f4(p0), d0 = ld_f4(p0 + 4), f1 = ld_f4(p1), d1 = ld_f4(p1 + 4);
+        f4 f;
+        f.x = fmaf(w3, d1.x, fmaf(w2, f1.x, fmaf(w1, d0.x, w0 * f0.x)));
+        f.y = fmaf(w3, d1.y, fmaf(w2, f1.y, fmaf(w1, d0.y, w0 * f0.y)));
+        f.z = fmaf(w3, d1.z, fmaf(w2, f1.z, fmaf(w1, d0.z, w0 * f0.z)));
+        f.w = fmaf(w3, d1.w, fmaf(w2, f1.w, fmaf(w1, d0.w, w0 * f0.w)));
+        st_f4(ew + (size_t)a * D::WP + 2 * D::H + 4 * q, f);
+    }
+}
 struct ZeroRows { float* p[64]; int n[64]; int count; };
 OARD_KERNEL __global__ __launch_bounds__(256) void k_zero_rows(ZeroRows z) {
     if ((int)blockIdx.x >= z.count) return;
diff --git a/oareactdiff_amd/csrc/oard_layout.h b/oareactdiff_amd/csrc/oard_layout.h
--- a/oareactdiff_amd/csrc/oard_layout.h
+++ b/oareactdiff_amd/csrc/oard_layout.h
@@ -51,6 +51,7 @@
     size_t c0row;
     size_t u0;
     size_t rbf_means, rbf_betas;
+    size_t rlw, dtt, dtf;
     size_t enc[OARD_MAX_OBJECTS], dec[OARD_MAX_OBJECTS];
     LayerOff layer[OARD_MAX_LAYERS];
     size_t head;
diff --git a/oareactdiff_amd/csrc/oard_plan.h b/oareactdiff_amd/csrc/oard_plan.h
--- a/oareactdiff_amd/csrc/oard_plan.h
+++ b/oareactdiff_amd/csrc/oard_plan.h
@@ -16,6 +16,7 @@
     int equi_l0_skip = 1;
     int gcl_msum = 1;
     int equi_rbf_table = 1;
+    int radial_table = 1;
 };
 
 enum GclShape {
@@ -40,6 +41,7 @@
     int num_layers;
     bool scratch;
     unsigned rbf_good = 0;
+    unsigned dist_good = 0;
 };
 struct FwdPlan {
     int num_layers;
@@ -53,6 +55,7 @@
     NodeForm node;
     bool l0_skip;
     bool rbf_table[16];
+    bool radial_table;
     const GclLayer& gcl_at(int l) const { return gcl[(l == 0 ? 1 : 0) | (l == num_layers - 1 ? 2 : 0)]; }
 };
 
@@ -98,6 +101,9 @@
 inline bool plan_rbf_wanted(const FwdPlanIn& in) {
     return !in.train && in.opt.equi_rbf_table && in.A > 0 && plan_equi_shape(in) == EQ_W8;
 }
+inline bool plan_dist_wanted(const FwdPlanIn& in) {
+    return !in.train && in.opt.radial_table && in.A > 0 && plan_equi_shape(in) == EQ_W8 && !(in.precision & OARD_PREC_GCL_BF16X3);
+}
 inline FwdPlan make_fwd_plan(FwdPlanIn in) {
     if (in.train) { in.opt.gcl_variant = in.opt.equi_variant = 2; in.opt.node_variant = 1; in.opt.gcl_skip = 1; }
     const FwdOptions& o = in.opt;
@@ -113,6 +119,7 @@
     p.l0_skip = !in.train && o.equi_l0_skip && in.A > 0 && p.node == NODE_LARGE && p.equi == EQ_W8;
     for (int l = 0; l < 16; ++l)
         p.rbf_table[l] = !in.train && o.equi_rbf_table && in.A > 0 && p.equi == EQ_W8 && l < in.num_layers && ((in.rbf_good >> l) & 1u);
+    p.radial_table = plan_dist_wanted(in) && (in.dist_good & 1u);
     auto throughput = [&](long long n) { const GclShape s = plan_gcl_shape(in, n); return n == 0 || s == GCL_PERSIST || s == GCL_RING3; };
     p.msum = !in.train && o.gcl_msum && in.E > 0 && o.gcl_variant == 2 && p.node == NODE_LARGE && throughput(in.CI) && throughput(in.CX);
     const long long inner = p.msum ? in.CI : in.A, all = p.msum ? in.CI + in.CX : in.E;
```

Result: no change. 3789 reaction-steps/s, median of 6 (+0.7%).
